# jacky121298/3DAL_PyTorch

Hardware: AMD Instinct MI355X
Metric: object-crops/sec through static+dynamic refinement heads (higher is better)
Workload: dtype f32; 1 GPU; StaticModelOneBoxEst forward+decode, 4096 crops x 1024 pts per GPU, fp32 (BASELINE.json configs[1]); items_per_gpu=4096, points_per_item=1024, sampler=device, parallelism=single GPU

## Files before the change

### 3dal_pytorch_amd/_hip.py

```python
import ctypes as C
import os

import numpy as np
import torch

_HERE = os.path.dirname(os.path.abspath(__file__))
LIB_PATH = os.path.join(_HERE, "lib3dal_hip.so")

OK, EINVAL, EWORKSPACE, EHIP = 0, -1, -2, -3
F32, BF16, F16, F16X3 = 0, 1, 2, 3
DTYPES = {"fp32": F32, "bf16": BF16, "fp16": F16, "f16x3": F16X3}
HEAD_INS_SEG, HEAD_STATIC_BOX_EST, HEAD_POINT_EMB, HEAD_BOX_EMB, HEAD_DYNAMIC_BOX_EST = range(5)
SAMPLER_DEVICE, SAMPLER_CHOICE = 0, 1
PHASE_SEG, PHASE_BOX, PHASE_ALL = 1, 2, 3

vp = C.c_void_p


class Layer(C.Structure):
    _fields_ = [("weight", vp), ("bias", vp), ("bn_weight", vp), ("bn_bias", vp), ("bn_mean", vp),
                ("bn_var", vp), ("c_in", C.c_int32), ("c_out", C.c_int32)]


class PackItem(C.Structure):
# ... 200 lines not shown
                ("out_indices", vp), ("out_key", vp), ("n_out", vp), ("status", vp), ("max_workgroups", C.c_int64),
                ("workspace", vp), ("workspace_bytes", C.c_size_t)]


class SpTableArgs(C.Structure):
    _fields_ = [("B", C.c_int64), ("in_shape", _i3), ("out_shape", _i3), ("kernel", _i3), ("stride", _i3), ("padding", _i3),
                ("reserved", C.c_int32), ("out_capacity", C.c_int64), ("n_out", vp), ("out_indices", vp), ("in_capacity", C.c_int64),
                ("n_in", vp), ("in_key", vp), ("in_pos", vp), ("table", vp), ("max_workgroups", C.c_int64)]


class SpConvArgs(C.Structure):
    _fields_ = [("taps", C.c_int32), ("c_in", C.c_int32), ("c_out", C.c_int32), ("relu", C.c_int32), ("center_tap", C.c_int32),
                ("reserved", C.c_int32), ("in_capacity", C.c_int64), ("x", vp), ("out_capacity", C.c_int64), ("n_out", vp),
                ("table", vp), ("packed", vp), ("residual", vp), ("y", vp), ("canvas", vp), ("out_indices", vp),
                ("canvas_B", C.c_int64), ("canvas_shape", _i3), ("reserved2", C.c_int32), ("status", vp),
                ("max_workgroups", C.c_int64)]


SP_WGRAD_SLICE = 1024


class SpTableTransposedArgs(C.Structure):
    _fields_ = [("B", C.c_int64), ("in_shape", _i3), ("out_shape", _i3), ("kernel", _i3), ("stride", _i3), ("padding", _i3),
                ("reserved", C.c_int32), ("in_capacity", C.c_int64), ("n_in", vp), ("in_indices", vp), ("out_capacity", C.c_int64),
                ("n_out", vp), ("out_key", vp), ("table", vp), ("max_workgroups", C.c_int64)]


class SpWgradArgs(C.Structure):
    _fields_ = [("taps", C.c_int32), ("c_in", C.c_int32), ("c_out", C.c_int32), ("reserved", C.c_int32), ("in_capacity", C.c_int64),
                ("x", vp), ("out_capacity", C.c_int64), ("n_out", vp), ("table", vp), ("dy", vp), ("dw", vp), ("db", vp),
                ("max_workgroups", C.c_int64), ("workspace", vp), ("workspace_bytes", C.c_size_t)]


ROI_OVERFLOW = 4096
ROI_MAX_TASKS, ROI_MAX_WIDTH = 16, 256
_f2 = C.c_float * 2


class BevGatherArgs(C.Structure):
    _fields_ = [("B", C.c_int64), ("H", C.c_int64), ("W", C.c_int64), ("C", C.c_int32), ("sample_index", C.c_int32), ("map", Map),
                ("n", C.c_int64), ("xy", vp), ("xy_stride", C.c_int64), ("sample", vp), ("pc_start", _f2), ("voxel_size", _f2),
                ("out_stride", C.c_float), ("points_per_row", C.c_int32), ("out", vp), ("out_row_stride", C.c_int64),
                ("out_col_offset", C.c_int64)]


class RoiShape(C.Structure):
    _fields_ = [("c_in", C.c_int32), ("n_shared", C.c_int32), ("n_cls", C.c_int32), ("n_reg", C.c_int32), ("shared", _i3),
                ("cls", _i3), ("reg", _i3), ("num_class", C.c_int32), ("code_size", C.c_int32)]


class RoiHeadArgs(C.Structure):
    _fields_ = [("shape", RoiShape), ("packed", vp), ("B", C.c_int64), ("M", C.c_int64), ("num_point", C.c_int32), ("C", C.c_int32),
                ("T", C.c_int32), ("box_cols", C.c_int32), ("K", C.c_int64), ("keep_stride", C.c_int64), ("boxes", vp), ("scores", vp),
                ("labels", vp), ("keep", vp), ("keep_count", vp), ("seg_offsets", vp), ("label_base", C.c_int32 * ROI_MAX_TASKS),
                ("bev", Map), ("H", C.c_int64), ("W", C.c_int64), ("pc_start", _f2), ("voxel_size", _f2), ("out_stride", C.c_float),
                ("rois", vp), ("roi_scores", vp), ("roi_features", vp), ("out_boxes", vp), ("out_scores", vp), ("out_labels", vp),
                ("out_counts", vp), ("out_features", vp), ("box_preds", vp), ("cls_preds", vp), ("status", vp), ("workspace", vp),
                ("workspace_bytes", C.c_size_t)]


ROI_NO_SAMPLE = 8192
ROI_CLS_SCORE = {"roi_iou": 0, "cls": 1}
ROI_TRAIN_MAX_M, ROI_TRAIN_MAX_R, ROI_TRAIN_MAX_G = 512, 512, 1024


class RoiTargetsArgs(C.Structure):
    _fields_ = [("B", C.c_int64), ("M", C.c_int64), ("R", C.c_int64), ("G", C.c_int64), ("code_size", C.c_int32),
                ("reserved0", C.c_int32), ("T", C.c_int32), ("reserved", C.c_int32), ("K", C.c_int64), ("keep_stride", C.c_int64),
                ("boxes", vp), ("scores", vp), ("labels", vp), ("keep", vp), ("keep_count", vp), ("seg_offsets", vp),
                ("label_base", C.c_int32 * ROI_MAX_TASKS), ("rois", vp), ("roi_scores", vp), ("roi_labels", vp), ("gt", vp),
                ("draws", vp), ("fg_per_image", C.c_int32), ("cls_score_type", C.c_int32), ("reg_fg_thresh", C.c_float),
                ("cls_fg_thresh", C.c_float), ("cls_bg_thresh", C.c_float), ("cls_bg_thresh_lo", C.c_float),
                ("cls_thresh_span", C.c_float), ("reserved2", C.c_float), ("hard_bg_ratio", C.c_double), ("slot", vp), ("sample", vp),
                ("out_rois", vp), ("out_labels", vp), ("out_scores", vp), ("gt_iou", vp), ("gt_src", vp), ("reg_valid", vp),
                ("cls_labels", vp), ("gt_of_rois", vp), ("out_boxes", vp), ("status", vp)]


CENTER_OVERFLOW = 16384
CENTER_MAX_OBJS, CENTER_MAX_CLASSES, CENTER_MAX_COLS = 1024, 64, 10
_pT = vp * ROI_MAX_TASKS


class CenterTargetsArgs(C.Structure):
    _fields_ = [("B", C.c_int64), ("G", C.c_int64), ("H", C.c_int64), ("W", C.c_int64), ("T", C.c_int32), ("max_objs", C.c_int32),
                ("num_class", C.c_int32 * ROI_MAX_TASKS), ("gt", vp), ("pc_start", _f2), ("voxel_size", _f2),
                ("out_size_factor", C.c_float), ("min_radius", C.c_int32), ("gaussian_overlap", C.c_double), ("hm", _pT),
                ("anno_box", _pT), ("ind", _pT), ("mask", _pT), ("cat", _pT), ("status", vp)]


class CenterLossArgs(C.Structure):
    _fields_ = [("B", C.c_int64), ("H", C.c_int64), ("W", C.c_int64), ("C", C.c_int32), ("n_cols", C.c_int32), ("max_objs", C.c_int32),
                ("reserved", C.c_int32), ("hm", Map), ("reg", Map), ("height", Map), ("dim", Map), ("rot", Map), ("vel", Map),
                ("target_hm", vp), ("anno_box", vp), ("ind", vp), ("mask", vp), ("cat", vp),
                ("code_weights", C.c_float * CENTER_MAX_COLS), ("weight", C.c_float), ("reserved2", C.c_float), ("out", vp),
                ("grad", vp), ("workspace", vp), ("workspace_bytes", C.c_size_t)]


AUG_TOO_MANY, AUG_OVERFLOW, AUG_BAD_ROW = 32768, 65536, 131072
AUG_MAX_BOXES, AUG_MAX_CAND = 1024, 64


class GtPasteArgs(C.Structure):
    _fields_ = [("B", C.c_int64), ("max_gt", C.c_int32), ("max_cand", C.c_int32), ("gt_boxes", vp), ("gt_classes", vp),
                ("gt_counts", vp), ("cand_boxes", vp), ("cand_group", vp), ("cand_counts", vp), ("accept", vp), ("coll", vp),
                ("status", vp)]


class AugmentPointsArgs(C.Structure):
    _fields_ = [("B", C.c_int64), ("n", C.c_int64), ("n_scene", C.c_int64), ("db_rows", C.c_int64), ("F", C.c_int32),
                ("transform", C.c_int32), ("max_cand", C.c_int64), ("scene", vp), ("scene_offsets", vp), ("db_points", vp),
                ("out_offsets", vp), ("cand_counts", vp), ("cand_seg_start", vp), ("cand_rows", vp), ("cand_db_row", vp),
                ("cand_boxes", vp), ("accept", vp), ("keys", vp), ("xform", vp), ("out", vp), ("status", vp),
                ("max_workgroups", C.c_int64), ("workspace", vp), ("workspace_bytes", C.c_size_t)]


class AugmentBoxesArgs(C.Structure):
    _fields_ = [("B", C.c_int64), ("max_gt", C.c_int32), ("max_cand", C.c_int32), ("max_objs", C.c_int32), ("n_classes", C.c_int32),
                ("transform", C.c_int32), ("reserved", C.c_int32), ("gt_boxes", vp), ("gt_classes", vp), ("gt_counts", vp),
                ("cand_boxes", vp), ("cand_classes", vp), ("cand_counts", vp), ("accept", vp), ("xform", vp),
                ("range", C.c_float * 4), ("out", vp), ("out_count", vp), ("status", vp)]


OPTIM_CHUNK, OPTIM_NORM_SPAN = 4096, 16384
OPTIM_TRUE_WD, OPTIM_CLIP, OPTIM_FUSED_ZERO = 1, 2, 4
(OPTIM_STEP, OPTIM_LR, OPTIM_BETA1, OPTIM_BETA2, OPTIM_EPS, OPTIM_WD, OPTIM_MAX_NORM, OPTIM_FLAGS, OPTIM_TOTAL_STEP,
 OPTIM_TABLE, OPTIM_SLOTS) = range(11)


class OptimChunk(C.Structure):
    _fields_ = [("param", vp), ("offset", C.c_int64), ("count", C.c_int32), ("decay", C.c_int32)]


_i, _i64, _u64, _sz = C.c_int, C.c_int64, C.c_uint64, C.c_size_t
SIGNATURES = {
    "dal3_version": (_i, []),
    "dal3_last_error": (C.c_char_p, []),
    "dal3_mean_size": (C.POINTER(C.c_float), []),
    "dal3_pack_weights": (_i, [_i, C.POINTER(Layer), _i, _i, vp, C.POINTER(_sz), vp]),
    "dal3_ins_seg_workspace_bytes": (_sz, [_i]),
    "dal3_ins_seg_plan_layout": (_i, [_i, C.POINTER(_sz), C.POINTER(_i)]),
    "dal3_ins_seg_encoder_route": (_i, [_i, _i, _i]),
    "dal3_ins_seg_forward": (_i, [vp, _i, _i, BCN, _i, _i, vp, vp, vp, vp, _sz, vp]),
    "dal3_ins_seg_encode": (_i, [vp, _i, _i, BCN, _i, _i, vp, vp]),
    "dal3_ins_seg_global_bias": (_i, [vp, _i, vp, _i, vp, vp]),
    "dal3_ins_seg_decode": (_i, [vp, _i, _i, BCN, _i, _i, vp, vp, vp, vp]),
    "dal3_gather_workspace_bytes": (_sz, [_i, _i]),
    "dal3_segment_counts": (_i, [vp, _i, _i, vp, vp]),
    "dal3_mask_compact_sample": (_i, [vp, BCN, _i, _i, _i, _i, _i, vp, _u64, _i64, vp, vp, vp, vp, _sz, vp]),
    "dal3_mask_compact_sample_step": (_i, [vp, BCN, _i, _i, _i, _i, _u64, vp, _i64, vp, vp, vp, vp, _sz, vp]),
    "dal3_point_head_workspace_bytes": (_sz, [_i]),
    "dal3_point_head_forward": (_i, [_i, vp, _i, BCN, _i, _i, vp, _i64, vp, _sz, vp]),
    "dal3_point_head_pool_workspace_bytes": (_sz, [_i, _i]),
    "dal3_point_head_screen_min_tiles": (_i, []),
    "dal3_point_head_screen_stride": (_i, []),
    "dal3_point_head_pool": (_i, [_i, vp, _i, BCN, _i, _i, vp, vp, vp, _sz, vp]),
    "dal3_dynamic_box_est_forward": (_i, [vp, vp, _i, vp, vp, _sz, vp]),
    "dal3_decode_boxes": (_i, [vp, _i, vp, _i64, _i, vp, _i64, vp, _i64, vp, vp, vp, vp, vp]),
    "dal3_recenter_rotz": (_i, [vp, _i, _i, vp, vp, vp, vp, vp, vp, vp]),
    "dal3_static_crop_prep": (_i, [vp, vp, vp, vp, vp, _i, _i, _u64, _i64, vp, vp, vp]),
    "dal3_dynamic_item_prep": (_i, [vp, vp, vp, vp, vp, vp, vp, vp, _i, _i, _i, _i, _u64, _i64, vp, vp, vp, vp]),
    "dal3_writeback_boxes": (_i, [vp, vp, vp, vp, vp, vp, vp, vp, vp, _i, _i64, vp, vp, vp]),
    "dal3_static_crop_labels": (_i, [vp, vp, vp, vp, _i, _i, _u64, _i64, vp, vp, vp]),
    "dal3_dynamic_item_labels": (_i, [vp, vp, vp, vp, vp, vp, vp, _i, _i, _i, _u64, _i64, vp, vp, vp, vp, vp]),
    "dal3_points_in_boxes": (_i, [vp, _i, _i64, _i64, vp, _i, _i, vp, vp]),
    "dal3_box_iou_pairwise": (_i, [vp, _i64, vp, _i64, _i, vp, vp, vp]),
    "dal3_box_iou_paired": (_i, [vp, vp, _i64, _i, vp, vp, vp]),
    "dal3_box_estimation_metrics": (_i, [C.POINTER(BoxMetricArgs), vp]),
    "dal3_track_workspace_bytes": (_sz, [_i64, _i64, _i64]),
    "dal3_track": (_i, [C.POINTER(TrackArgs), vp]),
    "dal3_track_match_workspace_bytes": (_sz, [_i64]),
    "dal3_track_match": (_i, [C.POINTER(TrackMatchArgs), vp]),
    "dal3_group_workspace_bytes": (_sz, [_i64, _i64]),
    "dal3_group_by_key": (_i, [C.POINTER(GroupArgs), vp]),
    "dal3_track_features": (_i, [C.POINTER(TrackFeatureArgs), vp]),
    "dal3_gt_table": (_i, [C.POINTER(GtTableArgs), vp]),
    "dal3_motion_classify_workspace_bytes": (_sz, [_i64]),
    "dal3_motion_classify": (_i, [C.POINTER(MotionClassifyArgs), vp]),
    "dal3_score_workspace_bytes": (_sz, [_i64]),
    "dal3_score_tracks": (_i, [C.POINTER(ScoreArgs), vp]),
    "dal3_best_gt_iou": (_i, [C.POINTER(BestGtArgs), vp]),
    "dal3_nms_workspace_bytes": (_sz, [_i64, _i]),
    "dal3_nms": (_i, [C.POINTER(NmsArgs), vp]),
    "dal3_center_decode_workspace_bytes": (_sz, [_i64, _i64, _i64]),
    "dal3_center_decode": (_i, [C.POINTER(CenterDecodeArgs), vp]),
    "dal3_center_decode_flip4_workspace_bytes": (_sz, [_i64, _i64, _i64]),
    "dal3_center_decode_flip4": (_i, [C.POINTER(CenterDecodeFlip4Args), vp]),
    "dal3_flip4_points": (_i, [vp, _i64, C.c_int32, vp, _i64, vp, vp, _i64, vp]),
    "dal3_voxelize_workspace_bytes": (_sz, [_i64, _i64]),
    "dal3_voxelize": (_i, [C.POINTER(VoxelizeArgs), vp]),
    "dal3_pillar_pack": (_i, [C.POINTER(Layer), _i, _i, C.c_double, vp, vp]),
    "dal3_pillar_features": (_i, [C.POINTER(PillarFeatureArgs), vp]),
    "dal3_pillar_scatter": (_i, [vp, vp, _i64, vp, _i, vp, _i64, _i64, _i64, vp]),
    "dal3_voxel_mean": (_i, [vp, vp, _i64, vp, _i, _i, vp, vp]),
    "dal3_conv2d_pack_floats": (_sz, [_i, _i, _i]),
    "dal3_conv2d_pack": (_i, [C.POINTER(Layer), _i, C.c_double, vp, vp]),
    "dal3_conv2d": (_i, [C.POINTER(Conv2dArgs), vp]),
    "dal3_sp_sort_workspace_bytes": (_sz, [_i64]),
    "dal3_sp_sort": (_i, [C.POINTER(SpSortArgs), vp]),
    "dal3_sp_downsample_workspace_bytes": (_sz, [_i64, _i]),
    "dal3_sp_downsample": (_i, [C.POINTER(SpDownsampleArgs), vp]),
    "dal3_sp_table": (_i, [C.POINTER(SpTableArgs), vp]),
    "dal3_sp_conv_pack_floats": (_sz, [_i, _i, _i]),
    "dal3_sp_conv_pack": (_i, [C.POINTER(Layer), _i, C.c_double, vp, vp, vp]),
    "dal3_sp_conv": (_i, [C.POINTER(SpConvArgs), vp]),
    "dal3_sp_table_transposed": (_i, [C.POINTER(SpTableTransposedArgs), vp]),
    "dal3_sp_wgrad_workspace_bytes": (_sz, [_i, _i, _i, _i64]),
    "dal3_sp_wgrad": (_i, [C.POINTER(SpWgradArgs), vp]),
    "dal3_bev_gather": (_i, [C.POINTER(BevGatherArgs), vp]),
    "dal3_box_points": (_i, [vp, _i64, _i, _i, vp, vp]),
    "dal3_roi_pack_floats": (_sz, [C.POINTER(RoiShape)]),
    "dal3_roi_pack": (_i, [C.POINTER(RoiShape), C.POINTER(Layer), _i, C.POINTER(C.c_double), vp, vp]),
    "dal3_roi_head_workspace_bytes": (_sz, [_i64, _i64, _i, _i, _i]),
    "dal3_roi_head": (_i, [C.POINTER(RoiHeadArgs), vp]),
    "dal3_roi_post": (_i, [vp, vp, vp, _i64, _i, vp, vp, vp]),
    "dal3_roi_targets": (_i, [C.POINTER(RoiTargetsArgs), vp]),
    "dal3_roi_loss": (_i, [vp, vp, _i64, _i, vp, vp, vp, C.POINTER(C.c_float), C.c_float, C.c_float, vp, vp, vp, vp]),
    "dal3_center_targets": (_i, [C.POINTER(CenterTargetsArgs), vp]),
    "dal3_center_loss_workspace_bytes": (_sz, [_i64, _i64, _i64, _i64]),
    "dal3_center_loss": (_i, [C.POINTER(CenterLossArgs), vp]),
    "dal3_gt_paste_select": (_i, [C.POINTER(GtPasteArgs), vp]),
    "dal3_augment_points_workspace_bytes": (_sz, [_i64, _i64]),
    "dal3_augment_points": (_i, [C.POINTER(AugmentPointsArgs), vp]),
    "dal3_augment_boxes": (_i, [C.POINTER(AugmentBoxesArgs), vp]),
    "dal3_optim_partials": (_i64, [_i64]),
    "dal3_optim_grad_norm": (_i, [vp, _i64, vp, vp, vp]),
    "dal3_optim_step": (_i, [vp, _i64, vp, vp, vp, _i64, vp, vp, vp]),
    "dal3_optim_total_norm": (_i, [vp, _i64, vp, vp]),
    "dal3_crop_workspace_bytes": (_sz, [_i64, _i64]),
    "dal3_crop_count": (_i, [vp, vp, vp, vp, vp, _i, _i64, _i64, vp, vp, _sz, vp]),
    "dal3_crop_fill": (_i, [vp, vp, vp, vp, vp, _i, _i64, _i64, vp, vp, vp, vp, vp, _i64, vp, _sz, vp]),
    "dal3_crop_starts": (_i, [vp, vp, _i64, vp, vp, vp]),
    "dal3_crop_starts_capped": (_i, [vp, vp, _i64, vp, vp, _i64, vp]),
    "dal3_tr_linear": (_i, [vp, _i64, _i, _i64, vp, vp, _i, vp, _i64, _i, vp, _i64, _i, vp, _i64, _i, vp, _sz, vp]),
    "dal3_tr_linear_workspace_bytes": (_sz, [_i, _i]),
    "dal3_tr_linear_pack_layout": (_i, [_i64, _i, _i64, _i, _i, _i]),
    "dal3_tr_pack_many": (_i, [vp, _i, vp]),
    "dal3_tr_linear_prepacked": (_i, [vp, _i64, _i, _i64, vp, vp, _i, vp, _i64, _i, vp, _i64, _i, vp, _i64, _i, vp, vp]),
    "dal3_tr_linear_x3_layout": (_i, [_i64, _i, _i64, _i, _i, _i]),
    "dal3_tr_linear_x3": (_i, [vp, _i64, _i, _i64, vp, vp, _i, vp, _i64, _i, vp, _i64, vp, vp, vp]),
    "dal3_tr_bnbwd_apply_amax": (_i, [vp, _i64, _i, _i64, vp, _i64, vp, vp, _i64, vp, vp, vp, vp, vp, vp, vp, vp, _i64, vp, vp]),
    "dal3_tr_colred_workspace_bytes": (_sz, [_i64, _i]),
    "dal3_tr_act_colsum": (_i, [vp, _i64, _i, _i64, vp, vp, _i, vp, _i64, vp, _sz, vp, vp]),
    "dal3_tr_colred": (_i, [vp, _i64, _i, _i64, _i, vp, _i64, vp, vp, _i64, vp, vp, vp, vp, vp, _sz, vp, vp]),
    "dal3_tr_pool_coef": (_i, [vp, vp, vp, vp, vp, vp, _i, _i, _i64, vp, vp, vp]),
    "dal3_tr_head2_forward": (_i, [vp, _i64, _i, _i64, vp, vp, _i, vp, _i64, _u64, vp, C.c_float, vp, _i64, vp, vp, vp]),
    "dal3_tr_head2_dgrad": (_i, [vp, _i64, _i, vp, _i64, _u64, vp, C.c_float, vp, _i64, vp, _i64, vp]),
    "dal3_tr_head2_dgrad_bnbwd": (_i, [vp, _i64, _i, vp, _i64, _u64, vp, C.c_float, vp, _i64, vp, _i64, vp, _i64, vp, vp, vp, vp, vp,
                                       vp, vp, vp, vp, vp, vp, _sz, vp]),
    "dal3_tr_head2_wgrad_workspace_bytes": (_sz, [_i64]),
    "dal3_tr_head2_wgrad": (_i, [vp, vp, _i64, _i, _i64, vp, vp, _i, vp, _i64, _u64, vp, C.c_float, vp, _sz, vp, vp]),
    "dal3_tr_conv1_workspace_bytes": (_sz, [_i64, _i]),
    "dal3_tr_conv1_bn_stats": (_i, [vp, _i64, _i64, _i, _i64, vp, _i64, vp, _i, vp, _i64, vp, vp, vp, vp, C.c_float, C.c_float, vp, vp,
                                    vp, vp, vp, _sz, vp]),
    "dal3_tr_conv1_wgrad": (_i, [vp, _i64, vp, _i64, _i, _i64, _i, vp, _sz, vp, vp]),
    "dal3_tr_gather_at": (_i, [vp, _i64, vp, _i64, _i, _i, vp, vp]),
    "dal3_tr_pool_zarg": (_i, [vp, vp, _i64, vp, _i64, vp, _i, _i, _i, _i, vp, vp]),
    "dal3_tr_pool_moments": (_i, [vp, _i64, vp, vp, vp, _i64, _i, _i, vp, vp]),
    "dal3_tr_pool_gv_workspace_bytes": (_sz, [_i]),
    "dal3_tr_pool_gv": (_i, [vp, vp, _i64, vp, _i, _i, vp, vp, vp, _sz, vp]),
    "dal3_tr_pool_dw": (_i, [vp, vp, _i64, vp, vp, vp, _i64, _i, vp, _i, _i, vp, vp]),
    "dal3_tr_pool_sparse": (_i, [vp, vp, vp, _i64, vp, _i64, _i, _i, _i, _i, vp, _i64, vp, vp]),
    "dal3_tr_box_loss": (_i, [vp] * 10 + [_i] + [vp] * 7),
    "dal3_tr_seg_ce_workspace_bytes": (_sz, [_i64]),
    "dal3_tr_seg_ce": (_i, [vp, vp, _i, _i64, vp, vp, vp, _sz, vp]),
    "dal3_tr_linear_red_workspace_bytes": (_sz, [_i64, _i]),
    "dal3_tr_linear_bn_stats": (_i, [vp, _i64, _i, _i64, vp, vp, _i, vp, _i64, vp, _i64, _i, vp, _i64, vp, _i64, vp, vp, vp, vp,
                                     C.c_float, C.c_float, vp, vp, vp, vp, vp, _sz, vp]),
    "dal3_tr_linear_bnbwd_sums": (_i, [vp, _i64, _i, _i64, vp, _i64, _i, vp, _i64, vp, _i64, vp, _i64, vp, vp, vp, vp, vp,
                                       vp, vp, vp, vp, vp, vp, _sz, vp]),
    "dal3_tr_bn_stats": (_i, [vp, _i64, _i, _i64, vp, vp, vp, vp, C.c_float, C.c_float, vp, vp, vp, vp, vp, _sz, vp]),
    "dal3_tr_bnbwd_sums": (_i, [vp, _i64, _i, _i64, vp, _i64, vp, vp, _i64, vp, vp, vp, vp, vp, vp, vp, vp, vp, vp, vp, _sz,
                                vp]),
    "dal3_tr_bn_finalize": (_i, [vp, _i, _i64, vp, vp, vp, vp, C.c_float, C.c_float, vp, vp, vp, vp, vp]),
    "dal3_tr_bnbwd_coef": (_i, [vp, _i, _i64, vp, vp, vp, vp, vp, vp, vp, vp]),
    "dal3_parse_box_pred": (_i, [vp, _i64, _i64, vp, vp, vp, vp, vp, vp, vp, vp]),
    "dal3_parse_box_pred_backward": (_i, [vp, vp, vp, vp, vp, vp, vp, _i64, vp, vp]),
    "dal3_tr_fc_max_rows": (_i, []),
    "dal3_tr_fc_max_act_cin": (_i, []),
    "dal3_tr_fc_forward": (_i, [vp, _i64, _i, _i64, vp, vp, _i, vp, _i64, _i, vp, _i, vp, _i64, vp, vp, vp, vp, C.c_float, C.c_float, vp, vp, vp, vp, vp]),
    "dal3_tr_fc_backward_w": (_i, [vp, _i64, _i64, _i, vp, _i64, vp, vp, vp, vp, vp, vp, vp, vp, _i, _i64, vp, vp, _i, vp, _i64, vp, _i64,
                                   vp, vp]),
    "dal3_tr_bnbwd_apply": (_i, [vp, _i64, _i, _i64, vp, _i64, vp, vp, _i64, vp, vp, vp, vp, vp, vp, vp, vp, _i64, vp]),
    "dal3_tr_bnbwd_apply_segsum_workspace_bytes": (_sz, [_i64, _i]),
    "dal3_tr_bnbwd_apply_segsum": (_i, [vp, _i64, _i, _i64, vp, _i64, vp, vp, vp, vp, vp, vp, vp, vp, _i64, _i64, vp, vp, _sz, vp]),
    "dal3_tr_wgrad_workspace_bytes": (_sz, [_i64, _i, _i]),
    "dal3_tr_wgrad": (_i, [vp, _i64, vp, _i64, vp, vp, _i, _i64, _i, _i, vp, _sz, vp, vp]),
    "dal3_tr_wgrad_final_many": (_i, [C.POINTER(WgradPart), _i, vp]),
    "dal3_tr_wgrad_x3_workspace_bytes": (_sz, [_i64, _i, _i]),
    "dal3_tr_wgrad_x3": (_i, [vp, _i64, vp, _i64, vp, vp, _i, vp, _i64, _i, _i, vp, _sz, vp, vp]),
    "dal3_tr_segmax": (_i, [vp, _i64, _i64, _i, vp, vp, vp, vp, _i64, vp, _sz, vp]),
    "dal3_tr_act_dropout": (_i, [vp, _i64, _i, _i64, vp, vp, _i, vp, _i64, _u64, vp, C.c_float, vp, _i64, vp]),
    "dal3_tr_linear_pool_workspace_bytes": (_sz, [_i, _i, _i64]),
    "dal3_tr_linear_pool": (_i, [vp, _i64, _i, _i64, vp, vp, _i, vp, _i64, vp, vp, vp, _i64, _i, vp, vp, vp, _sz, vp]),
    "dal3_tr_linear_pool_x3": (_i, [vp, _i64, _i, _i64, vp, vp, _i, vp, _i64, vp, vp, vp, _i64, _i, vp, vp, vp, _sz, vp]),
    "dal3_tr_linear_pool_x3_ok": (_i, [_i64, _i, _i64, _i]),
    "dal3_tr_segsum": (_i, [vp, _i64, _i64, _i, vp, _i64, vp]),
    "dal3_maxpool_n": (_i, [vp, _i64, _i64, vp, vp]),
    "dal3_maxpool_n_dtype": (_i, [vp, _i, _i64, _i64, vp, vp]),
    "dal3_shared_mlp_layer": (_i, [C.POINTER(Layer), _i, BCN, _i, _i, vp, vp, _sz, vp]),
    "dal3_shared_mlp_layer_workspace_bytes": (_sz, [_i, _i]),
    "dal3_static_workspace_bytes": (_sz, [_i, _i, _i]),
    "dal3_static_forward": (_i, [C.POINTER(StaticArgs), _i, vp]),
    "dal3_dynamic_workspace_bytes": (_sz, [_i, _i, _i]),
    "dal3_dynamic_forward": (_i, [C.POINTER(DynamicArgs), _i, vp]),
}

_lib = None


def lib():
    global _lib
    if _lib is None:
        if not os.path.exists(LIB_PATH):
            raise RuntimeError(
                f"{LIB_PATH} is missing: build the HIP library first "
                "(`make -C 3dal_pytorch_amd/csrc` or __graft_entry__.build()). "
                "There is no CPU/eager fallback for the eval-mode forward.")
        handle = C.CDLL(LIB_PATH)
        for name, (res, args) in SIGNATURES.items():
            fn = getattr(handle, name)
            fn.restype = res
            fn.argtypes = args
        from . import arch
        lib_mean = [handle.dal3_mean_size()[i] for i in range(9)]
        want = [C.c_float(v).value for row in arch.MEAN_SIZE for v in row]
        if lib_mean != want:
            raise RuntimeError(f"lib3dal_hip.so was built with MEAN_SIZE {lib_mean}, arch.MEAN_SIZE is {want}: rebuild the library")
        _lib = handle
    return _lib


def check(rc):
    if rc != OK:
        raise RuntimeError(f"lib3dal_hip error {rc}: {lib().dal3_last_error().decode()}")


def stream():
    return vp(torch.cuda.current_stream().cuda_stream)


def ptr(t):
    return vp(t.data_ptr()) if t is not None else vp(None)


def require_gpu(t, what):
    if not t.is_cuda:
        raise RuntimeError(
            f"{what} lives on {t.device}: the eval-mode forward runs only on an MI355X through "
            "lib3dal_hip.so (no CPU fallback). Move the model and its inputs to the GPU.")


def workspace(nbytes, device):
    return torch.empty(max(int(nbytes), 8), dtype=torch.uint8, device=device)


def host_offsets(offsets, n, name, sized_by, count):
    if torch.is_tensor(offsets):
        if offsets.is_cuda:
            raise TypeError(f"{name} must be on the host (a list, an array or a CPU tensor): {sized_by} from it, and "
                            "reading a device tensor back would be the synchronisation this call avoids")
        offsets = offsets.numpy()
    off = np.ascontiguousarray(np.asarray(offsets, dtype=np.int64).reshape(-1))
    if off.size < 1:
        raise ValueError(f"{name} needs {count} + 1 entries")
    if off[0] < 0 or off[-1] > n or np.any(np.diff(off) < 0):
        raise ValueError(f"{name} must be non-decreasing within [0, {n}]")
    return off


STORAGE = {torch.float32: F32, torch.bfloat16: BF16, torch.float16: F16}
BCN_NO_SMALL_JOB_KERNELS, BCN_NO_WORKLIST, BCN_NO_LDS_SAMPLER = 1, 2, 4
BCN_NO_DEC_PLAN = 16
BCN_NO_ENC_RESIDENT = 32
ENC_ROUTE_LATENCY, ENC_ROUTE_DENSE, ENC_ROUTE_TWO_LAUNCH, ENC_ROUTE_RESIDENT = 0, 1, 2, 3
DISPATCH_FLAGS = 0


def bcn(t):
    assert t.dim() == 3 and t.dtype in STORAGE
    sb, sc, sn = t.stride()
    return BCN(ptr(t), sb, sc, sn, STORAGE[t.dtype], DISPATCH_FLAGS)


def layer_struct(conv, bn):
    w = conv.weight
    c_in, c_out = getattr(conv, "in_channels", w.shape[1]), getattr(conv, "out_channels", w.shape[0])
    if not w.is_contiguous() or w.dtype != torch.float32:
        raise RuntimeError("weights must be contiguous fp32")
    L = Layer(ptr(w), ptr(conv.bias), None, None, None, None, c_in, c_out)
    if bn is not None:
        L.bn_weight, L.bn_bias = ptr(bn.weight), ptr(bn.bias)
        L.bn_mean, L.bn_var = ptr(bn.running_mean), ptr(bn.running_var)
    return L


def fold_layer_struct(conv, bn, what="the layer's parameters"):
    ts = [conv.weight] + ([conv.bias] if conv.bias is not None else [])
    if bn is not None:
        ts += [bn.weight, bn.bias, bn.running_mean, bn.running_var]
    for t in ts:
        require_gpu(t, what)
        if t.dtype != torch.float32 or not t.is_contiguous():
            raise RuntimeError("weights must be contiguous fp32")
    return layer_struct(conv, bn)


F16_MAX = 65504.0


def check_f16x3_range(pairs):
    with torch.no_grad():
        worst = None
        for conv, bn in pairs:
            w = conv.weight.detach().reshape(conv.weight.shape[0], -1).abs().amax(1)
            if bn is not None:
                w = w * (bn.weight.detach() / torch.sqrt(bn.running_var.detach() + 1e-5)).abs()
            m = w.max()
            worst = m if worst is None else torch.maximum(worst, m)
        if worst is not None and not float(worst) < F16_MAX:
            raise ValueError(f"precision 'f16x3': a folded weight of magnitude {float(worst):.3g} is beyond fp16's range "
                             f"({F16_MAX:g}); this head cannot run on the f16x3 kernels (use precision 'fp32')")


def pack(head_kind, pairs, device, dtype=F32):
    if dtype == F16X3:
        check_f16x3_range(pairs)
    arr = (Layer * len(pairs))(*[layer_struct(c, b) for c, b in pairs])
    need = _sz(0)
    check(lib().dal3_pack_weights(head_kind, arr, len(pairs), dtype, None, C.byref(need), None))
    buf = torch.empty(need.value, dtype=torch.uint8, device=device)
    assert buf.data_ptr() % 256 == 0
    check(lib().dal3_pack_weights(head_kind, arr, len(pairs), dtype, ptr(buf), C.byref(need), stream()))
    return buf
```

### 3dal_pytorch_amd/csrc/dal3_api.hip

```cpp
#include <stdarg.h>
#include <stdio.h>
#include <string.h>

#include <type_traits>

#include "dal3_block.h"
#include "dal3_kernels.h"
#include "dal3_lp.h"

static thread_local char g_err[512] = "";

static int fail(int code, const char* fmt, ...) {
    va_list ap;
    va_start(ap, fmt);
    vsnprintf(g_err, sizeof(g_err), fmt, ap);
    va_end(ap);
    return code;
}

#define HIP_TRY(expr)                                                                           \
    do {                                                                                        \
        hipError_t e_ = (expr);                                                                 \
        if (e_ != hipSuccess) return fail(DAL3_EHIP, "%s: %s", #expr, hipGetErrorString(e_)); \
    } while (0)
// ... 215 lines not shown
    const bool lp = dtype != DAL3_F32 && !x3;
    size_t floats;
    switch (head_kind) {
        case DAL3_HEAD_INS_SEG:
            floats = x3 ? measure(ins_seg_16_walk<InsSegX3W>) + DAL3_BLOB_TAIL_FLOATS
                        : lp ? measure(ins_seg_16_walk<InsSegLpW>) : measure(ins_seg_walk) + DAL3_BLOB_TAIL_FLOATS;
            break;
        case DAL3_HEAD_STATIC_BOX_EST:
        case DAL3_HEAD_POINT_EMB:
        case DAL3_HEAD_BOX_EMB:
            floats = x3 ? measure(point_head_16_walk, head_kind, true) + DAL3_BLOB_TAIL_FLOATS
                        : lp ? measure(point_head_16_walk, head_kind, false)
                             : measure(point_head_walk, head_kind) + DAL3_BLOB_TAIL_FLOATS;
            break;
        case DAL3_HEAD_DYNAMIC_BOX_EST: floats = measure(fc_head_walk); break;
        default: return fail(DAL3_EINVAL, "dal3_pack_weights: unknown head_kind %d", head_kind);
    }
    const size_t need = floats * sizeof(float);
    if (!packed_dev) {
        *bytes_inout = need;
        return 0;
    }
    if (*bytes_inout < need) return fail(DAL3_EWORKSPACE, "dal3_pack_weights: need %zu bytes, got %zu", need, *bytes_inout);
    if (!L) return fail(DAL3_EINVAL, "dal3_pack_weights: layers is NULL");
    if (reinterpret_cast<uintptr_t>(packed_dev) & 255) return fail(DAL3_EINVAL, "packed_dev must be 256-byte aligned");
    hipStream_t s = static_cast<hipStream_t>(stream);
    HIP_TRY(hipMemsetAsync(packed_dev, 0, need, s));

    if (head_kind == DAL3_HEAD_INS_SEG) {
        if (n_layers != 10) return fail(DAL3_EINVAL, "ins_seg expects 10 layers, got %d", n_layers);
        const int c_in = L[0].c_in;
        if (c_in != 3 && c_in != 4) return fail(DAL3_EINVAL, "ins_seg c_in must be 3 or 4, got %d", c_in);
        static const int co[10] = {64, 64, 64, 128, 1024, 512, 256, 128, 128, 2};
        static const int ci[10] = {0, 64, 64, 64, 128, 1088, 512, 256, 128, 128};
        for (int i = 0; i < 10; ++i) TRY(check_layer(L[i], i == 0 ? c_in : ci[i], co[i], "ins_seg layer"));
        const int64_t F = 512;
        if (x3) {
            const InsSegX3W w = view(packed_dev, ins_seg_16_walk<InsSegX3W>);
            uint16_t* enc = const_cast<uint16_t*>(w.enc_stream);
            uint16_t* dec = const_cast<uint16_t*>(w.dec_stream);
            TRY(pack_ins_seg_16_open(L, c_in, w, true, s));
            HIP_TRY(launch_pack_weight_x3(L[1], 0, 0, 64, 2, 2, enc, s));
            HIP_TRY(launch_pack_weight_x3(L[2], 0, 0, 64, 2, 2, enc + 16 * F, s));
            HIP_TRY(launch_pack_weight_x3(L[3], 0, 0, 64, 4, 2, enc + 32 * F, s));
            HIP_TRY(launch_pack_weight_x3(L[4], 0, 0, 128, 32, 4, enc + 64 * F, s));
            HIP_TRY(launch_pack_weight_x3(L[1], 0, 0, 64, 2, 2, dec, s));
            HIP_TRY(launch_pack_weight_x3(L[5], 0, 0, 64, 16, 2, dec, s, PackGroups{2, 16 * F, 24 * F, 40 * F}));
            HIP_TRY(launch_pack_weight_x3(L[6], 1, 0, 512, 8, 16, dec, s, PackGroups{8, 32 * F, 72 * F, 40 * F, 624 * F}));
            HIP_TRY(launch_pack_weight_x3(L[7], 0, 0, 256, 4, 8, dec + 656 * F, s));
            HIP_TRY(launch_pack_weight_x3(L[8], 0, 0, 128, 4, 4, dec + 784 * F, s));
            HIP_TRY(launch_pack_weight_x3(L[9], 0, 0, 128, 1, 4, dec + 848 * F, s));
            return 0;
        }
        if (lp) {
            const InsSegLpW w = view(packed_dev, ins_seg_16_walk<InsSegLpW>);
            uint16_t* enc = const_cast<uint16_t*>(w.enc_stream);
            uint16_t* dec = const_cast<uint16_t*>(w.dec_stream);
            TRY(pack_ins_seg_16_open(L, c_in, w, false, s));
            HIP_TRY(launch_pack_weight_lp(L[1], dtype, 0, 0, 64, 2, 2, enc, s));
            HIP_TRY(launch_pack_weight_lp(L[2], dtype, 0, 0, 64, 2, 2, enc + 8 * F, s));
            HIP_TRY(launch_pack_weight_lp(L[3], dtype, 0, 0, 64, 4, 2, enc + 16 * F, s));
            HIP_TRY(launch_pack_weight_lp(L[4], dtype, 0, 0, 128, 32, 4, enc + 32 * F, s));
            HIP_TRY(launch_pack_weight_lp(L[1], dtype, 0, 0, 64, 2, 2, dec, s));
            HIP_TRY(launch_pack_weight_lp(L[5], dtype, 0, 0, 64, 16, 2, dec, s, PackGroups{2, 8 * F, 40 * F, 20 * F}));
            HIP_TRY(launch_pack_weight_lp(L[6], dtype, 1, 0, 512, 8, 16, dec, s, PackGroups{8, 44 * F, 64 * F, 20 * F}));
            HIP_TRY(launch_pack_weight_lp(L[7], dtype, 0, 0, 256, 4, 8, dec, s, PackGroups{16, 360 * F, 400 * F, 40 * F}));
            HIP_TRY(launch_pack_weight_lp(L[8], dtype, 0, 0, 128, 4, 4, dec + 440 * F, s));
            HIP_TRY(launch_pack_weight_lp(L[9], dtype, 0, 0, 128, 1, 4, dec + 472 * F, s));
            return 0;
        }
        const InsSegW w = view(packed_dev, ins_seg_walk);
        HIP_TRY(launch_pack_weight(L[0], PACK_FIRST, 0, c_in, 2, 2, mut(w.w1), s));
        HIP_TRY(launch_pack_bias(L[0], mut(w.b1), s));
        TRY(pack_frag(L[1], PACK_FRAG_MT_MAJOR, 0, 64, w.enc_stream, ENC_W2, w.b2, s));
        TRY(pack_frag(L[2], PACK_FRAG_MT_MAJOR, 0, 64, w.enc_stream, ENC_W3, w.b3, s));
        TRY(pack_frag(L[3], PACK_FRAG_MT_MAJOR, 0, 64, w.enc_stream, ENC_W4, w.b4, s));
        TRY(pack_frag(L[4], PACK_FRAG_MT_MAJOR, 0, 128, w.enc_stream, ENC_W5, w.b5, s));
        TRY(pack_frag(L[1], PACK_FRAG_MT_MAJOR, 0, 64, w.dec_stream, DEC_W2, nullptr, s));
        TRY(pack_frag(L[5], PACK_FRAG_MT_MAJOR, 0, 64, w.dec_stream, DEC_MIX, w.db1, s,
                      PackGroups{ 2, 0, 8 * 256, 40 * 256}));
        HIP_TRY(launch_pack_weight(L[5], PACK_ROWMAJOR, 64, 1024, 0, 0, mut(w.dw1g), s));
        TRY(pack_frag(L[6], PACK_FRAG_KT_MAJOR, 0, 512, w.dec_stream, DEC_MIX, w.db2, s,
                      PackGroups{ 8, 16 * 256, 56 * 256, 40 * 256}));
        TRY(pack_frag(L[7], PACK_FRAG_MT_MAJOR, 0, 256, w.dec_stream, DEC_W3, w.db3, s));
        TRY(pack_frag(L[8], PACK_FRAG_MT_MAJOR, 0, 128, w.dec_stream, DEC_W4, w.db4, s));
        TRY(pack_frag(L[5], PACK_FRAG_MT_MAJOR, 0, 64, w.lat_stream, LAT_W1A, nullptr, s));
        TRY(pack_frag(L[6], PACK_FRAG_MT_MAJOR, 0, 512, w.lat_stream, LAT_W2, nullptr, s));
        HIP_TRY(launch_pack_weight(L[9], PACK_ROWMAJOR, 0, 128, 0, 0, mut(w.dw5), s));
        HIP_TRY(launch_pack_bias(L[9], mut(w.db5), s));
        HIP_TRY(launch_pack_weight(L[4], PACK_ROWMAJOR, 0, 128, 0, 0, mut(w.w5row), s));
        HIP_TRY(launch_pack_weight_lp(L[4], DAL3_F16, 0, 0, 128, 32, 4, reinterpret_cast<uint16_t*>(mut(w.w5h)), s));
        HIP_TRY(launch_pack_screen_bound(L[4], mut(w.scr_pq), const_cast<int32_t*>(w.scr_flag), s));
        int32_t* dec_flag = const_cast<int32_t*>(w.dec_flag);
        HIP_TRY(launch_pack_dec_chain(L[6], w.db2, mut(w.dw2c), dec_flag, s));
        HIP_TRY(launch_pack_dec_chain(L[7], w.db3, mut(w.dw3c), dec_flag, s));
        HIP_TRY(launch_pack_dec_chain(L[8], w.db4, mut(w.dw4c), dec_flag, s));
        HIP_TRY(launch_pack_weight_lp(L[5], DAL3_F16, 0, 0, 64, 16, 2, reinterpret_cast<uint16_t*>(mut(w.w1h)), s));
        HIP_TRY(launch_pack_dec_prune(L[5], mut(w.dw1c), mut(w.prn_pq), const_cast<uint32_t*>(w.dec_ident),
                                      const_cast<int32_t*>(w.prn_flag), s));
        return 0;
    }
    if (head_kind == DAL3_HEAD_DYNAMIC_BOX_EST) {
        if (n_layers != 3) return fail(DAL3_EINVAL, "dynamic box_est expects 3 layers, got %d", n_layers);
        return pack_fc(L, view(packed_dev, fc_head_walk), s);
    }
    int c_in, ks, c[4], n_fc, fi[3], fo[3];
    point_head_dims(head_kind, &c_in, &ks, c, &n_fc, fi, fo);
    if (n_layers != 4 + n_fc) return fail(DAL3_EINVAL, "head %d expects %d layers, got %d", head_kind, 4 + n_fc, n_layers);
    TRY(check_layer(L[0], c_in, c[0], "conv1"));
    for (int i = 1; i < 4; ++i) TRY(check_layer(L[i], c[i - 1], c[i], "conv"));
    if (x3 || lp) {
        const PointHeadLpW w = view(packed_dev, point_head_16_walk, head_kind, x3);
        TRY(pack_head_open(L, c_in, ks, c[0], w.w1, w.b1, w.bias, w.bias + c[1], w.bias + c[1] + c[2], s));
        uint16_t* st = const_cast<uint16_t*>(w.stream);
        const int64_t SEGE = (int64_t)LP_HEAD_SEG * 512;
        int64_t off = 0;
        int seg = 0;
        for (int l = 1; l < 4; ++l) {
            const int kt = c[l - 1] / 32, mt = c[l] / 32;
            if (x3) {
                HIP_TRY(launch_pack_weight_x3(L[l], 0, 0, c[l - 1], mt, kt, st + off, s));
                off += (int64_t)mt * kt * 2048;
            } else {
                const int tps = lp_tps(kt, mt);
                HIP_TRY(launch_pack_weight_lp(L[l], dtype, 0, 0, c[l - 1], mt, kt, st, s,
                                              PackGroups{tps * kt, seg * SEGE, (seg + 1) * SEGE, SEGE}));
                seg += mt / tps;
            }
        }
        return pack_fc(L + 4, w.fc, s);
    }
    const PointHeadW w = view(packed_dev, point_head_walk, head_kind);
    TRY(pack_head_open(L, c_in, ks, c[0], w.w1, w.b1, w.b2, w.b3, w.b4, s));
    const int f3 = (c[1] / 32) * (c[0] / 32) * 4, f4 = f3 + (c[2] / 32) * (c[1] / 32) * 4;
    TRY(pack_frag(L[1], PACK_FRAG_MT_MAJOR, 0, c[0], w.stream, 0, nullptr, s));
    TRY(pack_frag(L[2], PACK_FRAG_MT_MAJOR, 0, c[1], w.stream, f3, nullptr, s));
    TRY(pack_frag(L[3], PACK_FRAG_MT_MAJOR, 0, c[2], w.stream, f4, nullptr, s));
    if (w.w4row) {
        HIP_TRY(launch_pack_weight(L[3], PACK_ROWMAJOR, 0, 256, 0, 0, mut(w.w4row), s));
        HIP_TRY(launch_pack_weight_lp(L[3], DAL3_F16, 0, 0, 256, 16, 8, reinterpret_cast<uint16_t*>(mut(w.w4h)), s));
        HIP_TRY(launch_pack_screen_bound(L[3], mut(w.scr_pq), const_cast<int32_t*>(w.scr_flag), s));
    }
    return pack_fc(L + 4, w.fc, s);
}

static BCN to_bcn(const dal3_bcn& t) { return BCN{t.data, t.stride_b, t.stride_c, t.stride_n, t.dtype, t.flags}; }

static int check_bcn(const dal3_bcn& t, const char* what) {
    if (!t.data) return fail(DAL3_EINVAL, "%s: null data pointer", what);
    if (t.stride_n <= 0 || t.stride_c <= 0) return fail(DAL3_EINVAL, "%s: strides must be positive", what);
    if (t.dtype != DAL3_F32 && t.dtype != DAL3_BF16 && t.dtype != DAL3_F16)
        return fail(DAL3_EINVAL, "%s: storage dtype %d is none of DAL3_F32 / DAL3_BF16 / DAL3_F16", what, t.dtype);
    if (t.dtype != DAL3_F32 && (reinterpret_cast<uintptr_t>(t.data) & 1)) return fail(DAL3_EINVAL, "%s: 16-bit data must be 2-byte aligned", what);
    if (t.flags & ~(DAL3_BCN_NO_SMALL_JOB_KERNELS | DAL3_BCN_NO_WORKLIST | DAL3_BCN_NO_LDS_SAMPLER | DAL3_BCN_NO_DEC_PLAN | DAL3_BCN_NO_ENC_RESIDENT)) return fail(DAL3_EINVAL, "%s: unknown bits in flags (%d)", what, t.flags);
    return 0;
}

static int check_extent(int64_t B, int64_t N, const char* what) {
    if (B <= 0 || N <= 0) return fail(DAL3_EINVAL, "%s: B and N must be positive (B=%lld N=%lld)", what, (long long)B, (long long)N);
    if (B > DAL3_MAX_ITEMS) return fail(DAL3_EINVAL, "%s: B=%lld items exceed DAL3_MAX_ITEMS (%d)", what, (long long)B, DAL3_MAX_ITEMS);
    if (N > DAL3_MAX_POINTS_PER_ITEM)
        return fail(DAL3_EINVAL, "%s: N=%lld points per item exceed DAL3_MAX_POINTS_PER_ITEM (%d)", what, (long long)N, DAL3_MAX_POINTS_PER_ITEM);
    if (B * ((N + 31) / 32) > (int64_t)DAL3_MAX_TILES)
        return fail(DAL3_EINVAL, "%s: B=%lld x N=%lld is %lld 32-point tiles, more than DAL3_MAX_TILES (%d): split the batch", what,
                    (long long)B, (long long)N, (long long)(B * ((N + 31) / 32)), DAL3_MAX_TILES);
    return 0;
}

struct InsSegWs { float* g; float* gb; uint32_t* prune; uint32_t* plan_k; float* plan_gbc; int32_t* plan_nch; };
static InsSegWs carve_ins_seg(Carver& c, int B) {
    InsSegWs w;
    w.g = c.take<float>((size_t)B * 1024);
    w.gb = c.take<float>((size_t)B * 512);
    w.prune = c.take<uint32_t>((size_t)B * 513);
    w.plan_k = c.take<uint32_t>((size_t)B * DEC_PLAN_LD);
    w.plan_gbc = c.take<float>((size_t)B * 512);
    w.plan_nch = c.take<int32_t>((size_t)B);
    return w;
}
extern "C" size_t dal3_ins_seg_workspace_bytes(int B) {
    Carver c(nullptr, 0);
    carve_ins_seg(c, B);
    return c.off;
}

extern "C" int dal3_ins_seg_plan_layout(int B, size_t off[4], int* min_dead) {
    if (B <= 0 || !off) return fail(DAL3_EINVAL, "ins_seg_plan_layout: bad argument");
    char* const origin = reinterpret_cast<char*>(uintptr_t(4096));
    Carver c(origin, ~size_t(0));
    const InsSegWs w = carve_ins_seg(c, B);
    off[0] = reinterpret_cast<char*>(w.prune) - origin, off[1] = reinterpret_cast<char*>(w.plan_k) - origin;
    off[2] = reinterpret_cast<char*>(w.plan_gbc) - origin, off[3] = reinterpret_cast<char*>(w.plan_nch) - origin;
    if (min_dead) *min_dead = DAL3_DEC_MIN_DEAD;
    return 0;
}

extern "C" int dal3_ins_seg_encoder_route(int B, int N, int flags) {
    TRY(check_extent(B, N, "ins_seg_encoder_route"));
    if (flags & ~(DAL3_BCN_NO_SMALL_JOB_KERNELS | DAL3_BCN_NO_WORKLIST | DAL3_BCN_NO_LDS_SAMPLER | DAL3_BCN_NO_DEC_PLAN | DAL3_BCN_NO_ENC_RESIDENT))
        return fail(DAL3_EINVAL, "ins_seg_encoder_route: unknown bits in flags (%d)", flags);
    return enc_route(flags, B, N);
}

static int check_dtype(int dtype) {
    if (dtype != DAL3_F32 && dtype != DAL3_BF16 && dtype != DAL3_F16 && dtype != DAL3_F16X3)
        return fail(DAL3_EINVAL, "unknown dtype %d", dtype);
    return 0;
}

static int ins_seg_run(const void* packed, int dtype, int c_in, const dal3_bcn& pts, int B, int N, float* logits,
                       uint8_t* mask, float* global_feat_out, const InsSegWs& ws, hipStream_t s) {
    TRY(check_dtype(dtype));
    if (!packed || !logits || !mask) return fail(DAL3_EINVAL, "ins_seg: null pointer");
    TRY(check_extent(B, N, "ins_seg"));
    if (c_in != 3 && c_in != 4) return fail(DAL3_EINVAL, "ins_seg: c_in must be 3 or 4");
    TRY(check_bcn(pts, "pts"));
    const BCN x = to_bcn(pts);
    HIP_TRY(launch_nonfinite_rows(x, B, N, c_in, ws.g, 1024, s));
    if (dtype == DAL3_F32) {
        const InsSegW w = view(packed, ins_seg_walk);
        const bool plan = dec_plan_route(x.flags, B, N);
        if (plan) HIP_TRY(hipMemsetAsync(ws.prune, 0, (size_t)B * 513 * sizeof(uint32_t), s));
        HIP_TRY(launch_ins_seg_encode(w, x, c_in, B, N, ws.g, s, plan ? ws.prune : nullptr));
        HIP_TRY(launch_fc(w.dw1g, w.db1, ws.g, 1024, ws.gb, 512, B, 1024, 512, 0, s));
        if (plan) HIP_TRY(launch_dec_plan(w, ws.gb, ws.prune, B, ws.plan_k, ws.plan_gbc, ws.plan_nch, s));
        HIP_TRY(launch_ins_seg_decode(w, x, c_in, B, N, ws.gb, logits, mask, s,
                                      plan ? DecPlan{ws.plan_k, ws.plan_gbc, ws.plan_nch} : DecPlan{nullptr, nullptr, nullptr}));
    } else if (dtype == DAL3_F16X3) {
        const InsSegX3W w = view(packed, ins_seg_16_walk<InsSegX3W>);
        HIP_TRY(launch_ins_seg_encode_x3(w, x, c_in, B, N, ws.g, s));
        HIP_TRY(launch_fc(w.dw1g, w.db1, ws.g, 1024, ws.gb, 512, B, 1024, 512, 0, s));
        HIP_TRY(launch_ins_seg_decode_x3(w, x, c_in, B, N, ws.gb, logits, mask, s));
    } else {
        const InsSegLpW w = view(packed, ins_seg_16_walk<InsSegLpW>);
        HIP_TRY(launch_ins_seg_encode_lp(dtype, w, x, c_in, B, N, ws.g, s));
        HIP_TRY(launch_fc(w.dw1g, w.db1, ws.g, 1024, ws.gb, 512, B, 1024, 512, 0, s));
        HIP_TRY(launch_ins_seg_decode_lp(dtype, w, x, c_in, B, N, ws.gb, logits, mask, s));
    }
    if (global_feat_out)
        HIP_TRY(hipMemcpyAsync(global_feat_out, ws.g, (size_t)B * 1024 * sizeof(float), hipMemcpyDeviceToDevice, s));
    return 0;
}

extern "C" int dal3_ins_seg_forward(const void* packed, int dtype, int c_in, dal3_bcn pts, int B, int N, float* logits,
                                    uint8_t* mask, float* global_feat_out, void* workspace, size_t workspace_bytes,
                                    dal3_stream stream) {
    if (!workspace) return fail(DAL3_EINVAL, "ins_seg: workspace is NULL");
    TRY(check_extent(B, N, "ins_seg"));
    Carver c(workspace, workspace_bytes);
    const InsSegWs ws = carve_ins_seg(c, B);
    if (!c.ok) return fail(DAL3_EWORKSPACE, "ins_seg: workspace needs %zu bytes, got %zu", c.off, workspace_bytes);
    return ins_seg_run(packed, dtype, c_in, pts, B, N, logits, mask, global_feat_out, ws, static_cast<hipStream_t>(stream));
}

extern "C" int dal3_ins_seg_encode(const void* packed, int dtype, int c_in, dal3_bcn pts, int B, int N,
                                   float* global_feat, dal3_stream stream) {
    TRY(check_dtype(dtype));
    if (!packed || !global_feat || (c_in != 3 && c_in != 4)) return fail(DAL3_EINVAL, "ins_seg_encode: bad argument");
    TRY(check_extent(B, N, "ins_seg_encode"));
    TRY(check_bcn(pts, "pts"));
    hipStream_t s = static_cast<hipStream_t>(stream);
    if (dtype == DAL3_F32)
        HIP_TRY(launch_ins_seg_encode(view(packed, ins_seg_walk), to_bcn(pts), c_in, B, N,
                                      global_feat, s));
    else if (dtype == DAL3_F16X3)
        HIP_TRY(launch_ins_seg_encode_x3(view(packed, ins_seg_16_walk<InsSegX3W>), to_bcn(pts), c_in, B, N, global_feat, s));
    else
        HIP_TRY(launch_ins_seg_encode_lp(dtype, view(packed, ins_seg_16_walk<InsSegLpW>), to_bcn(pts), c_in, B, N, global_feat, s));
    return 0;
}

extern "C" int dal3_ins_seg_global_bias(const void* packed, int dtype, const float* global_feat, int B, float* gbias,
                                        dal3_stream stream) {
    TRY(check_dtype(dtype));
    if (!packed || !global_feat || !gbias) return fail(DAL3_EINVAL, "ins_seg_global_bias: bad argument");
    TRY(check_extent(B, 1, "ins_seg_global_bias"));
    const float *dw1g, *db1;
    auto sections = [&](const auto& w) { dw1g = w.dw1g, db1 = w.db1; };
    if (dtype == DAL3_F32) sections(view(packed, ins_seg_walk));
    else if (dtype == DAL3_F16X3) sections(view(packed, ins_seg_16_walk<InsSegX3W>));
    else sections(view(packed, ins_seg_16_walk<InsSegLpW>));
    HIP_TRY(launch_fc(dw1g, db1, global_feat, 1024, gbias, 512, B, 1024, 512, 0, static_cast<hipStream_t>(stream)));
    return 0;
}

extern "C" int dal3_ins_seg_decode(const void* packed, int dtype, int c_in, dal3_bcn pts, int B, int N,
                                   const float* gbias, float* logits, uint8_t* mask, dal3_stream stream) {
    TRY(check_dtype(dtype));
    if (!packed || !gbias || !logits || !mask || (c_in != 3 && c_in != 4)) return fail(DAL3_EINVAL, "ins_seg_decode: bad argument");
    TRY(check_extent(B, N, "ins_seg_decode"));
    TRY(check_bcn(pts, "pts"));
    hipStream_t s = static_cast<hipStream_t>(stream);
    if (dtype == DAL3_F32)
        HIP_TRY(launch_ins_seg_decode(view(packed, ins_seg_walk), to_bcn(pts), c_in, B, N,
                                      gbias, logits, mask, s));
    else if (dtype == DAL3_F16X3)
        HIP_TRY(launch_ins_seg_decode_x3(view(packed, ins_seg_16_walk<InsSegX3W>), to_bcn(pts), c_in, B, N, gbias, logits, mask, s));
    else
        HIP_TRY(launch_ins_seg_decode_lp(dtype, view(packed, ins_seg_16_walk<InsSegLpW>), to_bcn(pts), c_in, B, N, gbias, logits, mask, s));
    return 0;
}

extern "C" size_t dal3_gather_workspace_bytes(int B, int N) {
    Carver c(nullptr, 0);
    c.take<int32_t>((size_t)B * N);
    return c.off;
}

extern "C" int dal3_segment_counts(const uint8_t* mask, int B, int N, int32_t* counts, dal3_stream stream) {
    if (!mask || !counts) return fail(DAL3_EINVAL, "segment_counts: bad argument");
    TRY(check_extent(B, N, "segment_counts"));
    HIP_TRY(launch_segment_counts(mask, B, N, counts, static_cast<hipStream_t>(stream)));
    return 0;
}

static int gather_run(const uint8_t* mask, const dal3_bcn& pts, int B, int N, int C, int M, int sampler,
                      const int32_t* choice, uint64_t seed, int64_t item_offset, int32_t* counts, int32_t* obj_idx,
                      float* obj_pts, int32_t* pos, hipStream_t s, const int64_t* step = nullptr) {
    if (!mask || !counts || !obj_idx || !obj_pts) return fail(DAL3_EINVAL, "gather: null pointer");
    if (M <= 0 || C <= 0 || C > 8) return fail(DAL3_EINVAL, "gather: bad shape");
    TRY(check_extent(B, N, "gather"));
    TRY(check_extent(B, M, "gather (object points)"));
    if (sampler == DAL3_SAMPLER_CHOICE && !choice) return fail(DAL3_EINVAL, "gather: DAL3_SAMPLER_CHOICE needs choice");
    if (sampler != DAL3_SAMPLER_CHOICE && sampler != DAL3_SAMPLER_DEVICE) return fail(DAL3_EINVAL, "gather: bad sampler");
    TRY(check_bcn(pts, "pts"));
    HIP_TRY(launch_compact_sample(mask, to_bcn(pts), B, N, C, M, sampler, choice, seed, item_offset, counts, pos,
                                  obj_idx, obj_pts, s, step));
    return 0;
}

extern "C" int dal3_mask_compact_sample(const uint8_t* mask, dal3_bcn pts, int B, int N, int C, int M, int sampler,
                                        const int32_t* choice, uint64_t seed, int64_t item_offset, int32_t* counts,
                                        int32_t* obj_idx, float* obj_pts, void* workspace, size_t workspace_bytes,
                                        dal3_stream stream) {
    if (!workspace) return fail(DAL3_EINVAL, "gather: workspace is NULL");
    TRY(check_extent(B, N, "gather"));
    Carver c(workspace, workspace_bytes);
    int32_t* pos = c.take<int32_t>((size_t)B * N);
    if (!c.ok) return fail(DAL3_EWORKSPACE, "gather: workspace needs %zu bytes, got %zu", c.off, workspace_bytes);
    return gather_run(mask, pts, B, N, C, M, sampler, choice, seed, item_offset, counts, obj_idx, obj_pts, pos,
                      static_cast<hipStream_t>(stream));
}

extern "C" int dal3_mask_compact_sample_step(const uint8_t* mask, dal3_bcn pts, int B, int N, int C, int M, uint64_t seed,
                                             const int64_t* step, int64_t item_offset, int32_t* counts, int32_t* obj_idx,
                                             float* obj_pts, void* workspace, size_t workspace_bytes, dal3_stream stream) {
    if (!workspace) return fail(DAL3_EINVAL, "gather: workspace is NULL");
    TRY(check_extent(B, N, "gather"));
    Carver c(workspace, workspace_bytes);
    int32_t* pos = c.take<int32_t>((size_t)B * N);
    if (!c.ok) return fail(DAL3_EWORKSPACE, "gather: workspace needs %zu bytes, got %zu", c.off, workspace_bytes);
    return gather_run(mask, pts, B, N, C, M, DAL3_SAMPLER_DEVICE, nullptr, seed, item_offset, counts, obj_idx, obj_pts, pos,
                      static_cast<hipStream_t>(stream), step);
}

#define HEAD_WORK_MAX_POINTS 2560
struct HeadWs { float* feat; float* t1; float* t2; void* work; size_t work_bytes; };
static HeadWs carve_head(Carver& c, int B) {
    HeadWs w;
    w.feat = c.take<float>((size_t)B * 512);
    w.t1 = c.take<float>((size_t)B * 512);
    w.t2 = c.take<float>((size_t)B * 512);
    w.work_bytes = point_head_worklist_bytes(B, HEAD_WORK_MAX_POINTS);
    w.work = c.take<char>(w.work_bytes);
    return w;
}
extern "C" size_t dal3_point_head_workspace_bytes(int B) {
    Carver c(nullptr, 0);
    carve_head(c, B);
    return c.off;
}

static int fc_chain(const FcW& f, const float* x, int64_t xs, float* out, int64_t out_stride, int B, float* t1,
                    float* t2, hipStream_t s, const DecodeArgs* dec = nullptr) {
    const float* cur = x;
    int64_t cs = xs;
    for (int i = 0; i < f.n; ++i) {
        const bool last = i == f.n - 1;
        float* dst = last ? out : (i % 2 == 0 ? t1 : t2);
        const int64_t ds = last ? out_stride : f.c_out[i];
        if (last && dec) {
            if (f.c_out[i] != 39 || out_stride != 39 || dec->box_pred != out || f.relu[i])
                return fail(DAL3_EINVAL, "fc_chain: a fused decode needs the 39-wide box_pred layer last");
            HIP_TRY(launch_fc39_decode(f.w[i], f.b[i], cur, cs, B, f.c_in[i], *dec, s));
            return 0;
        }
        HIP_TRY(launch_fc(f.w[i], f.b[i], cur, cs, dst, ds, B, f.c_in[i], f.c_out[i], f.relu[i], s));
        cur = dst;
        cs = ds;
    }
    return 0;
}

static int point_head_run(int head_kind, const void* packed, int dtype, const dal3_bcn& x, int B, int M, float* out,
                          int64_t out_stride, const HeadWs& ws, hipStream_t s, const int32_t* distinct = nullptr,
                          const DecodeArgs* dec = nullptr) {
    TRY(check_dtype(dtype));
    if (head_kind != DAL3_HEAD_STATIC_BOX_EST && head_kind != DAL3_HEAD_POINT_EMB && head_kind != DAL3_HEAD_BOX_EMB)
        return fail(DAL3_EINVAL, "point_head: head_kind %d is not a point head", head_kind);
    if (!packed || !out) return fail(DAL3_EINVAL, "point_head: null pointer");
    TRY(check_extent(B, M, "point_head"));
    TRY(check_bcn(x, "x"));
    int c_in, ks, c[4], n_fc, fi[3], fo[3];
    point_head_dims(head_kind, &c_in, &ks, c, &n_fc, fi, fo);
    if (dtype == DAL3_F16X3) {
        const PointHeadX3W w = view(packed, point_head_16_walk, head_kind, true);
        HIP_TRY(launch_point_head_x3(head_kind, w, to_bcn(x), c_in, B, M, ws.feat, distinct, s));
        return fc_chain(w.fc, ws.feat, 512, out, out_stride, B, ws.t1, ws.t2, s, dec);
    }
    if (dtype != DAL3_F32) {
        const PointHeadLpW w = view(packed, point_head_16_walk, head_kind, false);
        HIP_TRY(launch_point_head_lp(dtype, head_kind, w, to_bcn(x), c_in, B, M, ws.feat, distinct, s));
        return fc_chain(w.fc, ws.feat, 512, out, out_stride, B, ws.t1, ws.t2, s, dec);
    }
    const PointHeadW w = view(packed, point_head_walk, head_kind);
    HIP_TRY(launch_point_head(head_kind, w, to_bcn(x), c_in, B, M, ws.feat, distinct, s, ws.work, ws.work_bytes));
    return fc_chain(w.fc, ws.feat, 512, out, out_stride, B, ws.t1, ws.t2, s, dec);
}

extern "C" int dal3_point_head_forward(int head_kind, const void* packed, int dtype, dal3_bcn x, int B, int M, float* out,
                                       int64_t out_stride, void* workspace, size_t workspace_bytes,
                                       dal3_stream stream) {
    if (!workspace) return fail(DAL3_EINVAL, "point_head: workspace is NULL");
    TRY(check_extent(B, M, "point_head"));
    Carver c(workspace, workspace_bytes);
    const HeadWs ws = carve_head(c, B);
    if (!c.ok) return fail(DAL3_EWORKSPACE, "point_head: workspace needs %zu bytes, got %zu", c.off, workspace_bytes);
    return point_head_run(head_kind, packed, dtype, x, B, M, out, out_stride, ws, static_cast<hipStream_t>(stream));
}

extern "C" size_t dal3_point_head_pool_workspace_bytes(int B, int M) {
    return B > 0 && M > 0 ? point_head_worklist_bytes(B, M) : 0;
}

extern "C" int dal3_point_head_pool(int head_kind, const void* packed, int dtype, dal3_bcn x, int B, int M,
                                    const int32_t* n_distinct, float* feat, void* workspace, size_t workspace_bytes,
                                    dal3_stream stream) {
    TRY(check_dtype(dtype));
    if (head_kind != DAL3_HEAD_STATIC_BOX_EST && head_kind != DAL3_HEAD_POINT_EMB && head_kind != DAL3_HEAD_BOX_EMB)
        return fail(DAL3_EINVAL, "point_head_pool: head_kind %d is not a point head", head_kind);
    if (!packed || !feat) return fail(DAL3_EINVAL, "point_head_pool: null pointer");
    if (workspace && (reinterpret_cast<uintptr_t>(workspace) & 15)) return fail(DAL3_EINVAL, "point_head_pool: workspace must be 16-byte aligned");
    TRY(check_extent(B, M, "point_head_pool"));
    TRY(check_bcn(x, "x"));
    hipStream_t s = static_cast<hipStream_t>(stream);
    int c_in, ks, c[4], n_fc, fi[3], fo[3];
    point_head_dims(head_kind, &c_in, &ks, c, &n_fc, fi, fo);
    if (dtype == DAL3_F16X3) {
        HIP_TRY(launch_point_head_x3(head_kind, view(packed, point_head_16_walk, head_kind, true), to_bcn(x), c_in, B, M, feat, n_distinct, s));
        return 0;
    }
    if (dtype != DAL3_F32) {
        const PointHeadLpW w = view(packed, point_head_16_walk, head_kind, false);
        HIP_TRY(launch_point_head_lp(dtype, head_kind, w, to_bcn(x), c_in, B, M, feat, n_distinct, s));
        return 0;
    }
    const PointHeadW w = view(packed, point_head_walk, head_kind);
    HIP_TRY(launch_point_head(head_kind, w, to_bcn(x), c_in, B, M, feat, n_distinct, s, workspace, workspace_bytes));
    return 0;
}

extern "C" int dal3_point_head_screen_min_tiles(void) { return DAL3_HEAD_SCREEN ? DAL3_HEAD_SCR_MIN_TILES : 0x7fffffff; }
extern "C" int dal3_point_head_screen_stride(void) { return DAL3_HEAD_SCR_STRIDE; }

extern "C" int dal3_dynamic_box_est_forward(const void* packed, const float* embedding, int B, float* box_pred,
                                            void* workspace, size_t workspace_bytes, dal3_stream stream) {
    if (!packed || !embedding || !box_pred || !workspace) return fail(DAL3_EINVAL, "dynamic_box_est: bad argument");
    TRY(check_extent(B, 1, "dynamic_box_est"));
    Carver c(workspace, workspace_bytes);
    const HeadWs ws = carve_head(c, B);
    if (!c.ok) return fail(DAL3_EWORKSPACE, "dynamic_box_est: workspace needs %zu bytes, got %zu", c.off, workspace_bytes);
    return fc_chain(view(packed, fc_head_walk), embedding, 384, box_pred, 39, B, ws.t1, ws.t2,
                    static_cast<hipStream_t>(stream));
}

extern "C" int dal3_decode_boxes(float* box_pred, int B, const float* center_add, int64_t center_add_stride,
                                 int center_inplace, const float* boxes_center_add, int64_t boxes_center_add_stride,
                                 const float* yaw_base, int64_t yaw_stride, float* heading_residuals,
                                 float* size_residuals, float* center, float* boxes7, dal3_stream stream) {
    if (!box_pred || B <= 0) return fail(DAL3_EINVAL, "decode_boxes: bad argument");
    HIP_TRY(launch_decode_boxes(box_pred, B, center_add, center_add_stride, center_inplace, boxes_center_add,
                                boxes_center_add_stride, yaw_base, yaw_stride, heading_residuals, size_residuals,
                                center, boxes7, static_cast<hipStream_t>(stream)));
    return 0;
}

extern "C" int dal3_recenter_rotz(const float* obj_pts, int B, int M, const float* init_box7, const float* box_one7,
                                  const float* bbox_gt7, float* obj_pts_two, int64_t* heading_class_label,
                                  float* heading_residual_label, dal3_stream stream) {
    if (!obj_pts || !init_box7 || !box_one7 || !obj_pts_two || B <= 0 || M <= 0)
        return fail(DAL3_EINVAL, "recenter_rotz: bad argument");
    if (bbox_gt7 && (!heading_class_label || !heading_residual_label))
        return fail(DAL3_EINVAL, "recenter_rotz: bbox_gt given without label outputs");
    HIP_TRY(launch_recenter(obj_pts, B, M, init_box7, box_one7, bbox_gt7, obj_pts_two, heading_class_label,
                            heading_residual_label, static_cast<hipStream_t>(stream)));
    return 0;
}

extern "C" int dal3_static_crop_prep(const double* points, const int64_t* offsets, const int32_t* choice,
                                     const double* pose, const double* box, int B, int N, uint64_t seed,
                                     int64_t item_offset, float* pts_out, float* init_box_out, dal3_stream stream) {
    if (!points || !offsets || !pose || !box || !pts_out || !init_box_out || B <= 0 || N < 7)
        return fail(DAL3_EINVAL, "static_crop_prep: bad argument (N must be >= 7)");
    HIP_TRY(launch_static_crop_prep(points, offsets, choice, pose, box, B, N, seed, item_offset, pts_out, init_box_out,
                                    static_cast<hipStream_t>(stream)));
    return 0;
}

extern "C" int dal3_dynamic_item_prep(const double* points, const int64_t* frame_offsets, const double* boxes,
                                      const int64_t* track_first, const int32_t* item_track, const int32_t* item_frame,
                                      const int32_t* choice, const double* pose, int B, int n_per, int r, int s,
                                      uint64_t seed, int64_t item_offset, float* pts_out, float* box_out,
                                      float* init_box_out, dal3_stream stream) {
    if (!points || !frame_offsets || !boxes || !track_first || !item_track || !item_frame || !pose || !pts_out ||
        !box_out || !init_box_out || B <= 0 || n_per <= 0 || r < 0 || s < 0)
        return fail(DAL3_EINVAL, "dynamic_item_prep: bad argument");
    HIP_TRY(launch_dynamic_item_prep(points, frame_offsets, boxes, track_first, item_track, item_frame, choice, pose, B,
                                     n_per, r, s, seed, item_offset, pts_out, box_out, init_box_out,
                                     static_cast<hipStream_t>(stream)));
    return 0;
}

extern "C" int dal3_static_crop_labels(const double* points, const int64_t* offsets, const int32_t* choice,
                                       const double* pose, int B, int N, uint64_t seed, int64_t item_offset,
                                       const double* gt_planes, uint8_t* mask_label, dal3_stream stream) {
    if (!points || !offsets || !pose || !gt_planes || !mask_label || B <= 0 || N <= 0)
        return fail(DAL3_EINVAL, "static_crop_labels: bad argument");
    HIP_TRY(launch_static_crop_labels(points, offsets, choice, pose, B, N, seed, item_offset, gt_planes, mask_label,
                                      static_cast<hipStream_t>(stream)));
    return 0;
}

extern "C" int dal3_dynamic_item_labels(const double* points, const int64_t* frame_offsets, const int64_t* track_first,
                                        const int32_t* item_track, const int32_t* item_frame, const int32_t* choice,
                                        const double* pose, int B, int n_per, int r, uint64_t seed, int64_t item_offset,
                                        const double* xform, const double* planes, const uint8_t* valid,
                                        uint8_t* mask_label, dal3_stream stream) {
    if (!points || !frame_offsets || !track_first || !item_track || !item_frame || !pose || !xform || !planes || !valid ||
        !mask_label || B <= 0 || n_per <= 0 || r < 0)
        return fail(DAL3_EINVAL, "dynamic_item_labels: bad argument");
    HIP_TRY(launch_dynamic_item_labels(points, frame_offsets, track_first, item_track, item_frame, choice, pose, B, n_per, r,
                                       seed, item_offset, xform, planes, valid, mask_label,
                                       static_cast<hipStream_t>(stream)));
    return 0;
}

extern "C" int dal3_points_in_boxes(const void* points, int points_f64, int64_t P, int64_t stride, const double* planes,
                                    int K, int f32_math, uint8_t* inside, dal3_stream stream) {
    if (P < 0 || K < 0 || stride < 3 || ((P > 0 && K > 0) && (!points || !planes || !inside)))
        return fail(DAL3_EINVAL, "points_in_boxes: bad argument (stride must be >= 3)");
    if (points_f64 && f32_math) return fail(DAL3_EINVAL, "points_in_boxes: float32 arithmetic needs float32 points");
    HIP_TRY(launch_points_in_boxes(points, points_f64, P, stride, planes, K, f32_math, inside,
                                   static_cast<hipStream_t>(stream)));
    return 0;
}

static int box_iou_args_ok(const char* what, const void* a, int64_t n, const void* b, int64_t m, int boxes_f64,
                           const float* iou_bev, const float* iou_3d, int64_t blocks) {
    if (n < 0 || m < 0 || (boxes_f64 != 0 && boxes_f64 != 1))
        return fail(DAL3_EINVAL, "%s: bad argument (n, m >= 0, boxes_f64 0 or 1)", what);
    if (n > DAL3_MAX_ITEMS || m > DAL3_MAX_ITEMS)
        return fail(DAL3_EINVAL, "%s: more than DAL3_MAX_ITEMS boxes on one side; split the call", what);
    if (blocks > DAL3_MAX_TILES) return fail(DAL3_EINVAL, "%s: launch grid beyond DAL3_MAX_TILES; split the call", what);
    if (!iou_bev && !iou_3d) return fail(DAL3_EINVAL, "%s: no output (iou_bev and iou_3d both NULL)", what);
    if (n > 0 && m > 0 && (!a || !b)) return fail(DAL3_EINVAL, "%s: null boxes", what);
    return 0;
}

extern "C" int dal3_box_iou_pairwise(const void* a, int64_t n, const void* b, int64_t m, int boxes_f64, float* iou_bev,
                                     float* iou_3d, dal3_stream stream) {
    const int64_t blocks = (n >= 0 && m >= 0 && n <= DAL3_MAX_ITEMS && m <= DAL3_MAX_ITEMS) ? box_iou_pairwise_blocks(n, m) : 0;
    TRY(box_iou_args_ok("box_iou_pairwise", a, n, b, m, boxes_f64, iou_bev, iou_3d, blocks));
    HIP_TRY(launch_box_iou_pairwise(a, n, b, m, boxes_f64, iou_bev, iou_3d, static_cast<hipStream_t>(stream)));
    return 0;
}

extern "C" int dal3_box_iou_paired(const void* a, const void* b, int64_t n, int boxes_f64, float* iou_bev, float* iou_3d,
                                   dal3_stream stream) {
    const int64_t blocks = (n >= 0 && n <= DAL3_MAX_ITEMS) ? box_iou_paired_blocks(n) : 0;
    TRY(box_iou_args_ok("box_iou_paired", a, n, b, n, boxes_f64, iou_bev, iou_3d, blocks));
    HIP_TRY(launch_box_iou_paired(a, b, n, boxes_f64, iou_bev, iou_3d, static_cast<hipStream_t>(stream)));
    return 0;
}

extern "C" int dal3_box_estimation_metrics(const dal3_box_metric_args* args, dal3_stream stream) {
    if (!args) return fail(DAL3_EINVAL, "box_estimation_metrics: null args");
    const dal3_box_metric_args& a = *args;
    if (a.B < 0 || a.N < 0 || a.B > DAL3_MAX_ITEMS || a.N > DAL3_MAX_POINTS_PER_ITEM)
        return fail(DAL3_EINVAL, "box_estimation_metrics: bad B / N (0 <= B <= DAL3_MAX_ITEMS, 0 <= N <= DAL3_MAX_POINTS_PER_ITEM)");
    if (!a.acc && !a.iou_bev && !a.iou_3d) return fail(DAL3_EINVAL, "box_estimation_metrics: no accumulator and no output");
    if ((a.f64_fields & ~255) || (a.i32_fields & ~3))
        return fail(DAL3_EINVAL, "box_estimation_metrics: unknown bits in f64_fields / i32_fields");
    if (a.B > 0) {
        const void* need[10] = {a.center, a.heading_scores, a.heading_residuals, a.size_scores, a.size_residuals,
                                a.center_label, a.heading_class_label, a.heading_residual_label, a.size_class_label,
                                a.size_residual_label};
        const int64_t ld[10] = {a.ld_center, a.ld_heading_scores, a.ld_heading_residuals, a.ld_size_scores,
                                a.ld_size_residuals, a.ld_center_label, a.ld_heading_class_label,
                                a.ld_heading_residual_label, a.ld_size_class_label, a.ld_size_residual_label};
        for (int k = 0; k < 10; ++k) {
            if (!need[k]) return fail(DAL3_EINVAL, "box_estimation_metrics: null field %d", k);
            if (ld[k] < 0) return fail(DAL3_EINVAL, "box_estimation_metrics: negative row stride of field %d", k);
        }
    }
    if (a.logits) {
        if (!a.acc) return fail(DAL3_EINVAL, "box_estimation_metrics: the segmentation term needs the accumulator");
        if (a.B > 0 && a.N > 0 && !a.mask_label) return fail(DAL3_EINVAL, "box_estimation_metrics: null mask_label");
        if (a.mask_dtype != DAL3_MASK_U8 && a.mask_dtype != DAL3_MASK_F32)
            return fail(DAL3_EINVAL, "box_estimation_metrics: mask_dtype must be DAL3_MASK_U8 or DAL3_MASK_F32");
        if (a.logits_stride_b < 0 || a.logits_stride_n < 0 || a.logits_stride_c < 0 || a.mask_stride_b < 0 ||
            a.mask_stride_n < 0)
            return fail(DAL3_EINVAL, "box_estimation_metrics: negative stride");
        if (1 + a.B * box_estimation_metrics_chunks(a.N) > DAL3_MAX_TILES)
            return fail(DAL3_EINVAL, "box_estimation_metrics: launch grid beyond DAL3_MAX_TILES; split the call");
    }
    HIP_TRY(launch_box_estimation_metrics(args, static_cast<hipStream_t>(stream)));
// ... 1709 lines not shown
```

### 3dal_pytorch_amd/csrc/dal3_head_screen.hip

```cpp
#include "dal3_device.h"
#include "dal3_kernels.h"
#include "dal3_lp.h"
#include "dal3_screen.h"

#ifndef HEAD_SCR_CAP
#define HEAD_SCR_CAP 1024
#endif
#define HEAD_SCR_XLD 132
#define HEAD_SCR_SW 16
#ifndef HEAD_SCR_DEPTH
#define HEAD_SCR_DEPTH 1
#endif
#define HEAD_SCR_XMAX_BITS 0x476A6000
#ifndef HEAD_RUN
#define HEAD_RUN 6
#endif

#ifdef DAL3_SCREEN_COUNT
__device__ unsigned long long g_head_scr_count[8];
extern "C" int dal3_debug_head_screen_counts(unsigned long long* out, int reset) {
    hipError_t e = hipMemcpyFromSymbol(out, HIP_SYMBOL(g_head_scr_count), sizeof(g_head_scr_count));
    if (e == hipSuccess && reset) {
        unsigned long long z[8] = {};
        e = hipMemcpyToSymbol(HIP_SYMBOL(g_head_scr_count), z, sizeof(z));
    }
    return (int)e;
}
#define HSCR_COUNT(k, v)                                                    \
    do {                                                                    \
        if (lane == 0) atomicAdd(&g_head_scr_count[k], (unsigned long long)(v)); \
    } while (0)
#else
#define HSCR_COUNT(k, v)
#endif

#ifdef DAL3_STAMP
__device__ unsigned long long* g_head_stamps = nullptr;
extern "C" int dal3_debug_set_head_stamps(void* p) {
    return (int)hipMemcpyToSymbol(HIP_SYMBOL(g_head_stamps), &p, sizeof(p));
}
#define HSTAMP_NOW(t)                                                               \
    do {                                                                            \
        __builtin_amdgcn_sched_barrier(0);                                          \
        asm volatile("s_memtime %0\n\ts_waitcnt lgkmcnt(0)" : "=s"(t)::"memory"); \
        __builtin_amdgcn_sched_barrier(0);                                          \
    } while (0)
#define HSTAMP(k)                                \
    do {                                         \
        unsigned long long t_;                   \
        HSTAMP_NOW(t_);                          \
        st_acc[k] += (uint32_t)(t_ - st_prev);   \
        st_prev = t_;                            \
    } while (0)
#define HSTAMP_ADD(k, v) st_acc[k] += (v)
#else
#define HSTAMP(k)
#define HSTAMP_ADD(k, v)
#endif

template <int KS, int C1, int C2, int C3>
__global__ __launch_bounds__(64) void point_head_screen_kernel(PointHeadW w, BCN x, int c_in, float* __restrict__ feat,
                                                               uint32_t* __restrict__ ctl, const u32x4* __restrict__ list) {
    constexpr int T = 1;
    constexpr int KT = C3 / 32;
    static_assert(C3 == 256, "the bound, the two halves of k and the fp16 fragments are laid out for conv4 256 -> 512");
    const int lane = threadIdx.x & 63;
    const int h = lane >> 5;
    __shared__ float s_b4[512];
    __shared__ int s_run[512];
    __shared__ int s_g[512];
    __shared__ f32x2 s_pq[512];
    __shared__ uint32_t s_list[HEAD_SCR_CAP];
    __shared__ float s_part[HEAD_SCR_CAP];
    __shared__ __attribute__((aligned(16))) float s_x[32 * HEAD_SCR_XLD];
    __shared__ __attribute__((aligned(16))) uint32_t s_stage[64 * (HEAD_SCR_SW + 4)];
    static_assert(4 * (3 * 512 * 4 + 512 * 8 + HEAD_SCR_CAP * 8 + 32 * HEAD_SCR_XLD * 4 + 64 * (HEAD_SCR_SW + 4) * 4) <= 160 * 1024,
                  "the screened head's LDS exceeds a quarter of a CU's 160 KiB: lower HEAD_SCR_CAP, HEAD_SCR_XLD or HEAD_SCR_SW");
    static_assert(16 * 64 <= 64 * (HEAD_SCR_SW + 4), "the stage holds the hit words of conv4's 16 blocks");
    for (int i = threadIdx.x; i < 512; i += 64) {
        s_b4[i] = w.b4[i];
        s_run[i] = 0;
        s_pq[i] = reinterpret_cast<const f32x2*>(w.scr_pq)[i];
    }
    __syncthreads();
    const uint32_t n_live = ctl[0];
    uint32_t run0 = n_live / (2u * gridDim.x);
    run0 = run0 < 1u ? 1u : (run0 > HEAD_RUN ? HEAD_RUN : run0);
    const uint32_t first_free = gridDim.x * run0;
    uint32_t cur = blockIdx.x * run0, run_end = cur + run0;
    if (cur >= n_live) return;
    const bool blob_dense = *w.scr_flag != 0;

    constexpr uint32_t FRAGS23 = ((C2 / 32) * (C1 / 32) + (C3 / 32) * (C2 / 32)) * 4u;
    WRing<DAL3_PF, true> ring;
    ring.init(w.stream, lane, FRAGS23 * 1024u);
    WRing<8> r16;
    r16.init(w.w4h, lane);
    f32x16 bias = tile_from_channels(w.b2, h);
    u32x4 e = list[cur];
    float in[T][KS];
    load_points<KS, T>(x, (int64_t)e[0], (int)e[1] * 32, (int)e[2], c_in, in, lane);
    auto enter = [&](int64_t b) {
        const int* gi = reinterpret_cast<const int*>(feat + b * 512);
#pragma unroll
        for (int c = lane; c < 512; c += 64) s_g[c] = __hip_atomic_load(gi + c, __ATOMIC_RELAXED, __HIP_MEMORY_SCOPE_AGENT);
    };
    auto flush = [&](int64_t b) {
        int* gi = reinterpret_cast<int*>(feat + b * 512);
#pragma unroll
        for (int c = lane; c < 512; c += 64) {
            const int v = s_run[c];
            if (v > 0) atomicMax(gi + c, v);
            s_run[c] = 0;
        }
    };
    auto dense_tile = [&](const f32x16 (&x3)[T][KT]) {
        WRing<DAL3_PF> r32;
        r32.init(w.stream + FRAGS23 * 64, lane);
        conv_max_layer<KT, T>(r32, s_b4, x3, reinterpret_cast<float*>(s_run), 16, lane);
    };
    enter((int64_t)e[0]);
#ifdef DAL3_STAMP
    uint32_t st_acc[10] = {};
    unsigned long long st_prev;
    HSTAMP_NOW(st_prev);
#endif
    for (;;) {
        const int64_t b = (int64_t)e[0];
        const int e_t = (int)e[1], e_n = (int)e[2];
        const bool last_of_run = cur + 1 >= run_end || cur + 1 >= n_live;
        uint32_t nxt = 0, take = 1;
        if (last_of_run) {
            const uint32_t left = n_live > run_end ? n_live - run_end : 0u;
            take = left / (2u * gridDim.x);
            take = take < 1u ? 1u : (take > HEAD_RUN ? HEAD_RUN : take);
            if (lane == 0) nxt = atomicAdd(&ctl[1], take);
        }
        f32x16 x3[T][KT];
        float in_n[T][KS];
        uint32_t ncur, nend;
        {
            f32x16 x1[T][C1 / 32], x2[T][C2 / 32];
            first_layer<KS, C1 / 32, T>(w.w1, w.b1, in, x1, lane);
            mlp_layer_ring<C1 / 32, C2 / 32, T>(ring, w.b2, w.b3, bias, x1, x2, lane);
            if (last_of_run) {
                ncur = (uint32_t)__builtin_amdgcn_readfirstlane((int)nxt) + first_free;
                nend = ncur + take;
            } else {
                ncur = cur + 1;
                nend = run_end;
            }
            const uint32_t nclamp = ncur < n_live ? ncur : cur;
            e = list[nclamp];
            mlp_layer_ring<C2 / 32, C3 / 32, T>(ring, w.b3, w.b2, bias, x2, x3, lane);
            load_points<KS, T>(x, (int64_t)e[0], (int)e[1] * 32, (int)e[2], c_in, in_n, lane);
        }
        HSCR_COUNT(0, 1);
        HSTAMP(0);
        HSTAMP_ADD(8, 1u);

        int xm = 0;
#pragma unroll
        for (int kt = 0; kt < KT; ++kt) {
#pragma unroll
            for (int r = 0; r < 16; ++r) {
                const int v = __float_as_int(x3[0][kt][r]);
                xm = v > xm ? v : xm;
            }
        }
        if (blob_dense || __builtin_amdgcn_ballot_w64(xm > HEAD_SCR_XMAX_BITS) != 0) {
            HSCR_COUNT(1, 1);
            dense_tile(x3);
            HSTAMP(7);
        } else {
            float ss = 0.0f;
#pragma unroll
            for (int kt = 0; kt < KT; ++kt) {
#pragma unroll
                for (int r = 0; r < 16; ++r) ss = fmaf(x3[0][kt][r], x3[0][kt][r], ss);
            }
            ss += __shfl_xor(ss, 32);
#pragma unroll
            for (int d = 16; d >= 1; d >>= 1) ss = __builtin_fmaxf(ss, __shfl_xor(ss, d));
            const float X = sqrtf(ss) * (1.0f + 0x1p-15f);

            ActTile<FP16> xh[KT];
#pragma unroll
            for (int kt = 0; kt < KT; ++kt) xh[kt] = pack_relu<FP16>(x3[0][kt]);

            ScreenHits<T> hits;
            hits.init();
            uint32_t vmask = 0;
            {
                const int left = e_n - e_t * 32;
#pragma unroll
                for (int r = 0; r < 16; ++r) vmask |= tile_chan(r, h) < left ? (1u << (15 - r)) : 0u;
            }
            HSTAMP(1);
            auto block_const = [&](int mt) -> float {
                const int c = 32 * mt + (lane & 31);
                const f32x2 pq = s_pq[c];
                float E = fmaf(X, pq[0], pq[1]);
                E = fmaf(E, 0x1p-20f, E);
                const int gs = s_g[c], gr = s_run[c];
                const float G = __int_as_float(gs > gr ? gs : gr), bb = s_b4[c];
                if (bits_nonfinite(G)) return 3.0e38f;
                return (G - bb) - fmaf(__builtin_fabsf(G) + __builtin_fabsf(bb), 0x1p-22f, E);
            };
            uint32_t hb = 0;
            auto ep_slice = [&](const f32x16& acc, int i, float k) {
                hb = scr_push_hit(hb, acc[2 * i], k);
                hb = scr_push_hit(hb, acc[2 * i + 1], k);
            };
            auto ep_finish = [&](int mt) {
                hits.park_block(s_stage, mt, hb & vmask, lane);
            };
            auto mm = [&](f32x16& acc, int mt, auto side) {
                acc = f32x16{};
#pragma unroll
                for (int i = 0; i < 2 * KT; ++i) {
                    const f16x8_t a = __builtin_bit_cast(f16x8_t, r16.slot[i & 7]);
                    r16.slot[i & 7] = r16.fetch_at(((16u * (uint32_t)mt + (uint32_t)i + 8u) & 255u) * 1024u);
                    acc = FP16::mfma(xh[i >> 1].k[i & 1], a, acc);
                    DAL3_SCHED_FENCE();
                    side(i);
                    DAL3_SCHED_FENCE();
                }
            };
            f32x16 accA, accB;
            float kA = block_const(0), kB;
            mm(accA, 0, NoSide());
            int mt = 1;
            for (; mt + 1 < 16; mt += 2) {
                kB = block_const(mt);
                mm(accB, mt, [&](int i) { if (i < 8) ep_slice(accA, i, kA); });
                ep_finish(mt - 1);
                kA = block_const(mt + 1);
                mm(accA, mt + 1, [&](int i) { if (i < 8) ep_slice(accB, i, kB); });
                ep_finish(mt);
            }
            kB = block_const(mt);
            mm(accB, mt, [&](int i) { if (i < 8) ep_slice(accA, i, kA); });
            ep_finish(mt - 1);
#pragma unroll
            for (int i = 0; i < 8; ++i) ep_slice(accB, i, kB);
            ep_finish(mt);
            HSTAMP(2);
            uint32_t cnt1[T];
            const bool overflow = scr_build_lists<T, 16, HEAD_SCR_CAP>(s_stage, s_list, hits, cnt1, lane);
            const uint32_t cnt = cnt1[0];
            HSCR_COUNT(3, cnt);
            HSTAMP(3);

            if (overflow) {
                HSCR_COUNT(2, 1);
                dense_tile(x3);
                HSTAMP(7);
            } else {
#pragma unroll
                for (int half = 0; half < 2; ++half) {
                    __builtin_amdgcn_wave_barrier();
#pragma unroll
                    for (int kt = 0; kt < 4; ++kt) {
#pragma unroll
                        for (int q = 0; q < 4; ++q) {
                            f32x4 v;
                            v[0] = x3[0][4 * half + kt][4 * q + 0];
                            v[1] = x3[0][4 * half + kt][4 * q + 1];
                            v[2] = x3[0][4 * half + kt][4 * q + 2];
                            v[3] = x3[0][4 * half + kt][4 * q + 3];
                            *reinterpret_cast<f32x4*>(s_x + (lane & 31) * HEAD_SCR_XLD + 32 * kt + 8 * q + 4 * h) = v;
                        }
                    }
                    __builtin_amdgcn_wave_barrier();
                    if (half == 1) HSCR_COUNT(4, (cnt + 63) / 64);
                    scr_recompute<HEAD_SCR_SW, 128 / HEAD_SCR_SW, HEAD_SCR_DEPTH, false>(
                        w.w4row + 128 * half, 256, s_list, cnt, s_x, HEAD_SCR_XLD, s_stage, lane,
                        [&](uint32_t idx, bool live) { return half == 0 ? 0.0f : s_part[live ? idx : 0u]; },
                        [&](float a, int c, uint32_t idx, bool live) {
                            if (half == 0) {
                                if (live) s_part[idx] = a;
                            } else {
                                int bits = __float_as_int(a + s_b4[c]);
                                bits = bits > 0 ? bits : 0;
                                if (live && bits > 0) atomicMax(&s_run[c], bits);
                            }
                        });
                    HSTAMP(4 + half);
                }
                HSTAMP_ADD(9, 1u);
            }
        }
        const bool more = ncur < n_live;
        const bool leave = !more || (int64_t)e[0] != b;
        if (leave) flush(b);
        HSTAMP(6);
        if (!more) break;
        if (leave) enter((int64_t)e[0]);
        HSTAMP(6);
        cur = ncur;
        run_end = nend;
#pragma unroll
        for (int k = 0; k < KS; ++k) in[0][k] = in_n[0][k];
    }
#ifdef DAL3_STAMP
    if (lane == 0 && blockIdx.x < 1024) {
#pragma unroll
        for (int k = 0; k < 10; ++k) g_head_stamps[blockIdx.x * 16 + k] = st_acc[k];
    }
#endif
}

hipError_t launch_point_head_screen(int head_kind, const PointHeadW& w, BCN x, int c_in, float* feat, uint32_t* ctl,
                                    const u32x4* list, int64_t max_tiles, int64_t slots, hipStream_t s) {
    if (!w.w4row || !w.w4h || !w.scr_pq || !w.scr_flag) return hipErrorInvalidValue;
    const dim3 grid((unsigned)(max_tiles < slots ? max_tiles : slots)), block(64);
    switch (head_kind) {
        case 1:
            hipLaunchKernelGGL((point_head_screen_kernel<2, 128, 128, 256>), grid, block, 0, s, w, x, c_in, feat, ctl, list);
            break;
        case 2:
            hipLaunchKernelGGL((point_head_screen_kernel<2, 64, 128, 256>), grid, block, 0, s, w, x, c_in, feat, ctl, list);
            break;
        default:
            return hipErrorInvalidValue;
    }
    return hipGetLastError();
}
```

### 3dal_pytorch_amd/csrc/dal3_kernels.h

```cpp
#pragma once
#include <hip/hip_runtime.h>
#include <stddef.h>
#include <stdint.h>

#include "../../include/dal3.h"
#include "dal3_device.h"
#include "dal3_fold.h"

#ifndef DAL3_ENC_T
#define DAL3_ENC_T 2
#endif
#ifndef DAL3_DEC_T
#define DAL3_DEC_T 1
#endif
#ifndef DAL3_HEAD_T
#define DAL3_HEAD_T 1
#endif

#ifndef DAL3_ENC_SCREEN
#define DAL3_ENC_SCREEN 1
#endif

#ifndef DAL3_WG_WAVES
#define DAL3_WG_WAVES 4
// ... 33 lines not shown
    const int32_t* scr_flag;
    const float* dw2c;
    const float* dw3c;
    const float* dw4c;
    const int32_t* dec_flag;
    const float* dw1c;
    const f32x4* w1h;
    const float* prn_pq;
    const uint32_t* dec_ident;
    const int32_t* prn_flag;
};
#ifndef DAL3_DEC_MIN_DEAD
#define DAL3_DEC_MIN_DEAD 64
#endif
#ifndef DAL3_DEC_PLAN_ROUND
#define DAL3_DEC_PLAN_ROUND 2
#endif
#define DEC_PLAN_LD 640
#define DEC_NULL_K 512
struct DecPlan {
    const uint32_t* k;
    const float* gbc;
    const int32_t* nch;
};
enum {
    ENC_W2 = 0, ENC_W3 = 16, ENC_W4 = 32, ENC_W5 = 64, ENC_FRAGS = 64 + 512,
    DEC_W2 = 0, DEC_MIX = 16, DEC_MIX_FRAGS = 8 + 16 * 40, DEC_W3 = 16 + 648, DEC_W4 = 16 + 648 + 128,
    DEC_FRAGS = 16 + 648 + 128 + 64,
    LAT_W1A = 0, LAT_W2 = 128, LAT_FRAGS = 128 + 512
};

struct PackGroups {
    int blocks = 0;
    int64_t a0 = 0, a1 = 0, stride = 0, last = -1;
};

struct FcW {
    const float* w[3];
    const float* b[3];
    int c_in[3], c_out[3], relu[3];
    int n;
};

struct PointHeadW {
    const float* w1;
    const float* b1;
    const float* b2;
    const float* b3;
    const float* b4;
    const f32x4* stream;
    FcW fc;
    const float* w4row;
    const f32x4* w4h;
    const float* scr_pq;
    const int32_t* scr_flag;
};

#define LP_ENC_SEG 32
#define LP_ENC_SEGS 9
#define LP_DEC_SEG 40
#define LP_DEC_SEGS 12
#define LP_HEAD_SEG 32
#ifndef DAL3_LP_ENC_T
#define DAL3_LP_ENC_T 4
#endif
#ifndef DAL3_LP_DEC_T
#define DAL3_LP_DEC_T 2
#endif
#ifndef DAL3_LP_HEAD_T
#define DAL3_LP_HEAD_T 2
#endif
struct InsSegLpW {
    const float* w1;
    const float* b1;
    const float* bias_enc;
    const float* bias_dec;
    const float* dw1g;
    const float* db1;
    const uint16_t* enc_stream;
    const uint16_t* dec_stream;
};
struct PointHeadLpW {
    const float* w1;
    const float* b1;
    const float* bias;
    const uint16_t* stream;
    FcW fc;
};
#ifndef DAL3_X3_HEAD_T
#define DAL3_X3_HEAD_T 2
#endif
#ifndef DAL3_X3_ENC_T
#define DAL3_X3_ENC_T 2
#endif
#ifndef DAL3_X3_DEC_T
#define DAL3_X3_DEC_T 2
#endif
typedef PointHeadLpW PointHeadX3W;
struct InsSegX3W {
    const float* w1;
    const float* b1;
    const float* bias_enc;
    const float* bias_dec;
    const float* dw1g;
    const float* db1;
    const uint16_t* enc_stream;
    const uint16_t* dec_stream;
};
hipError_t launch_ins_seg_encode_x3(const InsSegX3W& w, BCN pts, int c_in, int B, int N, float* g, hipStream_t s);
hipError_t launch_ins_seg_decode_x3(const InsSegX3W& w, BCN pts, int c_in, int B, int N, const float* gbias, float* logits,
                                    uint8_t* mask, hipStream_t s);
int point_head_x3_segments(int head_kind);
hipError_t launch_point_head_x3(int head_kind, const PointHeadX3W& w, BCN x, int c_in, int B, int M, float* feat,
                                const int32_t* distinct, hipStream_t s);
hipError_t launch_pack_weight_x3(const dal3_layer& L, int kt_major, int col_off, int n_cols, int mt_n, int kt_n, uint16_t* out,
                                 hipStream_t s, PackGroups G = PackGroups{});
hipError_t launch_ins_seg_encode_lp(int dtype, const InsSegLpW& w, BCN pts, int c_in, int B, int N, float* g, hipStream_t s);
hipError_t launch_ins_seg_decode_lp(int dtype, const InsSegLpW& w, BCN pts, int c_in, int B, int N, const float* gbias,
                                    float* logits, uint8_t* mask, hipStream_t s);
hipError_t launch_point_head_lp(int dtype, int head_kind, const PointHeadLpW& w, BCN x, int c_in, int B, int M,
                                float* feat, const int32_t* distinct, hipStream_t s);
hipError_t launch_pack_weight_lp(const dal3_layer& L, int dtype, int kt_major, int col_off, int n_cols, int mt_n, int kt_n,
                                 uint16_t* out, hipStream_t s, PackGroups G = PackGroups{});

void point_head_dims(int head_kind, int* c_in, int* ks, int c[4], int* n_fc, int fc_in[3], int fc_out[3]);

hipError_t launch_ins_seg_encode(const InsSegW& w, BCN pts, int c_in, int B, int N, float* g, hipStream_t s, uint32_t* prune = nullptr);
hipError_t launch_ins_seg_encode_screen(const InsSegW& w, BCN pts, int c_in, int B, int N, float* g, hipStream_t s, uint32_t* prune);
bool dec_plan_route(int flags, int B, int N);
int enc_route(int flags, int B, int N);
bool enc_resident_route(int flags, int B, int N);
hipError_t launch_pack_dec_prune(const dal3_layer& L, float* dw1c, float* pq, uint32_t* ident, int32_t* flag, hipStream_t s);
hipError_t launch_dec_plan(const InsSegW& w, const float* gb, const uint32_t* prune, int B, uint32_t* plan_k, float* plan_gbc,
                           int32_t* plan_nch, hipStream_t s);
hipError_t launch_pack_screen_bound(const dal3_layer& L, float* pq, int32_t* flag, hipStream_t s);
hipError_t launch_pack_dec_chain(const dal3_layer& L, const float* bias, float* wcopy, int32_t* flag, hipStream_t s);
hipError_t launch_ins_seg_decode(const InsSegW& w, BCN pts, int c_in, int B, int N, const float* gbias,
                                 float* logits, uint8_t* mask, hipStream_t s, DecPlan plan = DecPlan{nullptr, nullptr, nullptr});
size_t point_head_worklist_bytes(int B, int M);
hipError_t launch_point_head(int head_kind, const PointHeadW& w, BCN x, int c_in, int B, int M, float* feat,
                             const int32_t* distinct, hipStream_t s, void* worklist = nullptr, size_t worklist_bytes = 0);
#ifndef DAL3_HEAD_SCR_STRIDE
#define DAL3_HEAD_SCR_STRIDE 4
#endif
#ifndef DAL3_HEAD_SCREEN
#define DAL3_HEAD_SCREEN 1
#endif
#ifndef DAL3_HEAD_SCR_MIN_TILES
#define DAL3_HEAD_SCR_MIN_TILES 8192
#endif
static_assert(DAL3_HEAD_SCR_STRIDE >= 2, "stride 1 leaves no tile to screen");
hipError_t launch_point_head_screen(int head_kind, const PointHeadW& w, BCN x, int c_in, float* feat, uint32_t* ctl,
                                    const u32x4* list, int64_t max_tiles, int64_t slots, hipStream_t s);
hipError_t launch_pack_head_screen(const dal3_layer& L, float* pq, int32_t* flag, hipStream_t s);
hipError_t launch_generic_layer(const f32x4* wf, const float* w1, const float* bias, int kt_n, int ks_n, int mt_n,
                                int relu, BCN x, int c_in, int B, int N, float* y, hipStream_t s);

hipError_t launch_fc(const float* W, const float* bias, const float* x, int64_t xs, float* y, int64_t ys, int B,
                     int c_in, int c_out, int relu, hipStream_t s);

enum { PACK_FRAG_MT_MAJOR = 0, PACK_FRAG_KT_MAJOR = 1, PACK_FIRST = 2, PACK_ROWMAJOR = 3 };
hipError_t launch_pack_weight(const dal3_layer& L, int mode, int col_off, int n_cols, int mt_n, int kt_n, float* out,
                              hipStream_t s, PackGroups G = PackGroups{});
hipError_t launch_pack_bias(const dal3_layer& L, float* out, hipStream_t s);

hipError_t launch_static_crop_prep(const double* points, const int64_t* offsets, const int32_t* choice, const double* pose,
                                   const double* box, int B, int N, uint64_t seed, int64_t item_offset, float* pts_out,
                                   float* init_box_out, hipStream_t s);
hipError_t launch_dynamic_item_prep(const double* points, const int64_t* frame_offsets, const double* boxes,
                                    const int64_t* track_first, const int32_t* item_track, const int32_t* item_frame,
                                    const int32_t* choice, const double* pose, int B, int n_per, int r, int s_,
                                    uint64_t seed, int64_t item_offset, float* pts_out, float* box_out,
                                    float* init_box_out, hipStream_t st);
hipError_t launch_static_crop_labels(const double* points, const int64_t* offsets, const int32_t* choice, const double* pose,
                                     int B, int N, uint64_t seed, int64_t item_offset, const double* gt_planes,
                                     uint8_t* mask_label, hipStream_t s);
hipError_t launch_dynamic_item_labels(const double* points, const int64_t* frame_offsets, const int64_t* track_first,
                                      const int32_t* item_track, const int32_t* item_frame, const int32_t* choice,
                                      const double* pose, int B, int n_per, int r, uint64_t seed, int64_t item_offset,
                                      const double* xform, const double* planes, const uint8_t* valid, uint8_t* mask_label,
                                      hipStream_t st);
size_t crop_workspace_bytes(int64_t K_total, int64_t max_points_per_frame);
hipError_t launch_crop_count(const float* points, const int64_t* point_offsets, const double* planes,
                             const float* spheres, const int64_t* box_offsets, int F, int64_t K_total, int64_t max_points_per_frame,
                             int64_t* counts, int32_t* cc, hipStream_t s);
hipError_t launch_crop_fill(const float* points, const int64_t* point_offsets, const double* planes,
                            const float* spheres, const int64_t* box_offsets, int F, int64_t K_total,
                            int64_t max_points_per_frame, const double* pose, const int64_t* counts,
                            const int64_t* box_start, const int32_t* cc, double* out_points, int32_t* out_index,
                            int64_t out_capacity, hipStream_t s);
hipError_t launch_crop_starts(const int64_t* counts, const int64_t* order, int64_t K, int64_t* box_start, int64_t* out_offsets,
                              int64_t out_capacity, hipStream_t s);
int64_t box_iou_pairwise_blocks(int64_t n, int64_t m);
int64_t box_iou_paired_blocks(int64_t n);
hipError_t launch_box_iou_pairwise(const void* a, int64_t n, const void* b, int64_t m, int boxes_f64, float* iou_bev,
                                   float* iou_3d, hipStream_t s);
hipError_t launch_box_iou_paired(const void* a, const void* b, int64_t n, int boxes_f64, float* iou_bev, float* iou_3d,
                                 hipStream_t s);
int64_t box_estimation_metrics_chunks(int64_t N);
hipError_t launch_box_estimation_metrics(const dal3_box_metric_args* a, hipStream_t s);
size_t track_workspace_bytes(int64_t S, int64_t K, int64_t capacity);
size_t track_match_workspace_bytes(int64_t K);
hipError_t launch_track(const dal3_track_args* a, hipStream_t s);
hipError_t launch_track_match(const dal3_track_match_args* a, hipStream_t s);
size_t group_workspace_bytes(int64_t E, int64_t T);
size_t motion_classify_workspace_bytes(int64_t T);
hipError_t launch_group_by_key(const dal3_group_args* a, hipStream_t s);
hipError_t launch_track_features(const dal3_track_feature_args* a, hipStream_t s);
hipError_t launch_gt_table(const dal3_gt_table_args* a, hipStream_t s);
hipError_t launch_motion_classify(const dal3_motion_classify_args* a, hipStream_t s);
size_t score_workspace_bytes(int64_t S);
hipError_t launch_score_tracks(const dal3_score_args* a, hipStream_t s);
hipError_t launch_best_gt_iou(const dal3_best_gt_args* a, hipStream_t s);
size_t nms_workspace_bytes(int64_t K, int boxes_f64);
hipError_t launch_nms(const dal3_nms_args* a, hipStream_t s);
size_t center_decode_workspace_bytes(int64_t B, int64_t H, int64_t W);
hipError_t launch_center_decode(const dal3_center_decode_args* a, hipStream_t s);
hipError_t launch_center_decode_flip4(const dal3_center_decode_flip4_args* a, hipStream_t s);
hipError_t launch_flip4_points(const float* points, int64_t N, int C, const int64_t* offsets, int64_t B, float* out,
                               int64_t* out_offsets, int64_t max_workgroups, hipStream_t s);
size_t voxelize_workspace_bytes(int64_t B, int64_t N);
hipError_t launch_voxelize(const dal3_voxelize_args* a, hipStream_t s);
hipError_t launch_pillar_pack(const dal3_layer* layers, int n_layers, double eps, float* out, hipStream_t s);
hipError_t launch_pillar_features(const dal3_pillar_feature_args* a, hipStream_t s);
hipError_t launch_pillar_scatter(const float* features, const int32_t* coordinates, int64_t P, const int64_t* n_pillars, int c_out,
                                 float* canvas, int64_t canvas_B, int64_t ny, int64_t nx, hipStream_t s);
hipError_t launch_voxel_mean(const float* voxels, const int32_t* num_points, int64_t P, const int64_t* n_pillars, int max_points,
                             int C, float* out, hipStream_t s);
size_t conv2d_pack_floats(int kind, int c_in, int c_out);
hipError_t launch_conv2d_pack(const FoldLayer& layer, int kind, float* out, hipStream_t s);
hipError_t launch_conv2d(const dal3_conv2d_args* a, hipStream_t s);
size_t sp_sort_workspace_bytes(int64_t capacity);
hipError_t launch_sp_sort(const dal3_sp_sort_args* a, hipStream_t s);
int sp_candidates(const int32_t* kernel, const int32_t* stride);
size_t sp_downsample_workspace_bytes(int64_t in_capacity, int candidates);
hipError_t launch_sp_downsample(const dal3_sp_downsample_args* a, hipStream_t s);
hipError_t launch_sp_table(const dal3_sp_table_args* a, hipStream_t s);
size_t sp_conv_pack_floats(int taps, int c_in, int c_out);
hipError_t launch_sp_conv_pack(const FoldLayer& layer, int taps, float* out, int32_t* status, hipStream_t s);
hipError_t launch_sp_conv(const dal3_sp_conv_args* a, hipStream_t s);
hipError_t launch_sp_table_transposed(const dal3_sp_table_transposed_args* a, hipStream_t s);
size_t sp_wgrad_workspace_bytes(int taps, int c_in, int c_out, int64_t out_capacity);
hipError_t launch_sp_wgrad(const dal3_sp_wgrad_args* a, hipStream_t s);
hipError_t launch_points_in_boxes(const void* points, int points_f64, int64_t P, int64_t stride, const double* planes,
                                  int K, int f32_math, uint8_t* inside, hipStream_t s);
hipError_t launch_writeback(const double* final_boxes, const int32_t* final_idx, const double* pose_best,
                            const double* pose_inv, const double* track_box, float* det, const int64_t* det_start,
                            const int32_t* det_count, const uint8_t* active, int P, int64_t n_det, int32_t* match,
                            int32_t* owner, hipStream_t s);
hipError_t launch_maxpool_n(const void* x, int dtype, int64_t rows, int64_t n, void* out, hipStream_t s);
hipError_t launch_segment_counts(const uint8_t* mask, int B, int N, int32_t* counts, hipStream_t s);
hipError_t launch_fill_words(void* p, size_t n_words, uint32_t value, hipStream_t s);
hipError_t launch_nonfinite_rows(BCN x, int B, int n_pts, int c_in, float* dst, int C, hipStream_t s,
                                 const int32_t* distinct = nullptr, void* worklist = nullptr, int seed_stride = 0);
hipError_t launch_compact_sample(const uint8_t* mask, BCN pts, int B, int N, int C, int M, int sampler,
                                 const int32_t* choice, uint64_t seed, int64_t item_offset, int32_t* counts,
                                 int32_t* pos, int32_t* obj_idx, float* obj_pts, hipStream_t s, const int64_t* step = nullptr);
struct DecodeArgs {
    float* box_pred;
    const float* center_add;
    int64_t ca_stride;
    int center_inplace;
    const float* boxes_center_add;
    int64_t bca_stride;
    const float* yaw_base;
    int64_t yaw_stride;
    float* heading_residuals;
    float* size_residuals;
    float* center;
    float* boxes7;
};
hipError_t launch_fc39_decode(const float* W, const float* bias, const float* x, int64_t xs, int B, int c_in,
                              const DecodeArgs& d, hipStream_t s);
hipError_t launch_decode_boxes(float* box_pred, int B, const float* center_add, int64_t center_add_stride,
                               int center_inplace, const float* boxes_center_add, int64_t boxes_center_add_stride,
                               const float* yaw_base, int64_t yaw_stride, float* heading_residuals,
                               float* size_residuals, float* center, float* boxes7, hipStream_t s);
hipError_t launch_recenter(const float* obj_pts, int B, int M, const float* init_box7, const float* box_one7,
                           const float* bbox_gt7, float* obj_pts_two, int64_t* hcl, float* hrl, hipStream_t s);

hipError_t launch_tr_linear(const float* a, int64_t M, int c_in, int64_t lda, const float* scale, const float* shift,
                            int relu_in, const float* W, int64_t ldw, int transpose_w, const float* bias, int64_t seg,
                            int c_out, float* z, int64_t ldz, int accumulate, float* ws, hipStream_t s, bool prepacked = false);
size_t tr_linear_workspace_bytes(int c_in, int c_out);
int tr_linear_pack_mtb(int64_t M, int c_in, int64_t seg, int c_out, int accumulate, int has_act);
hipError_t launch_tr_pack_many(const dal3_tr_pack_item* items, int n, hipStream_t s);
int tr_linear_x3_layout(int64_t M, int c_in, int64_t seg, int c_out, int accumulate, int has_act);
hipError_t launch_tr_linear_x3(const float* a, int64_t M, int c_in, int64_t lda, const float* scale, const float* shift, int relu_in,
                               const uint16_t* wpk, int layout, const float* bias, int64_t seg, int c_out, float* z, int64_t ldz,
                               hipStream_t s, const uint32_t* in_amax = nullptr);
size_t tr_colred_workspace_bytes(int64_t M, int C);
hipError_t launch_tr_act_colsum(const float* x, int64_t M, int C, int64_t ldx, const float* scale, const float* shift, int relu,
                                float* out, int64_t ldo, double* part, double* sums, hipStream_t s);
hipError_t launch_tr_colred(const float* z, int64_t M, int C, int64_t ldz, int mode, const float* da, int64_t ldda,
                            const float* dg, const int32_t* arg, int64_t seg, const float* scale, const float* shift,
                            const float* mu, const float* rstd, double* part, double* out, hipStream_t s);
hipError_t launch_tr_pool_coef(const float* dg, const float* g, const float* zarg, const float* mu, const float* rstd,
                               const float* gamma, int B, int C, int64_t M, double* coef, float* kd, hipStream_t s);
hipError_t launch_tr_pool_moments(const float* W, int64_t ldw, const float* b, const double* m1, const float* Sc, int64_t M, int C,
                                  int K, double* sums, hipStream_t s);
__attribute__((visibility("hidden"))) bool tr_pool_k_ok(int K);
__attribute__((visibility("hidden"))) bool tr_conv1_ok(int c_in, int c_out);
size_t tr_pool_gv_workspace_bytes(int K);
hipError_t launch_tr_pool_gv(const double* coef, const float* W, int64_t ldw, const float* b, int C, int K, float* G, float* v,
                             double* ws, hipStream_t s);
hipError_t launch_tr_pool_dw(const double* coef, const float* W, int64_t ldw, const float* b, const float* S, const double* m1,
// ... 146 lines not shown
```

### 3dal_pytorch_amd/csrc/dal3_pointmlp.hip

```cpp
#include <stdlib.h>

#include <type_traits>

#include "dal3_device.h"
#include "dal3_kernels.h"

#ifdef DAL3_STAMP
__device__ long long* g_stamps = nullptr;
extern "C" int dal3_debug_set_stamps(void* p) {
    return (int)hipMemcpyToSymbol(HIP_SYMBOL(g_stamps), &p, sizeof(p));
}
#define STAMP(k)                                                                                  \
    do {                                                                                          \
        __builtin_amdgcn_sched_barrier(0);                                                        \
        unsigned long long t_;                                                                    \
        asm volatile("s_memtime %0\n\ts_waitcnt lgkmcnt(0)" : "=s"(t_)::"memory");               \
        __builtin_amdgcn_sched_barrier(0);                                                        \
        if (lane == 0 && blockIdx.x < 2048) g_stamps[(blockIdx.x * DAL3_WG_WAVES + wave) * 16 + (k)] = t_; \
    } while (0)
#else
#define STAMP(k)
#endif

#ifndef DAL3_ENC_LDS_MAX
// ... 700 lines not shown
            mlp_layer_ring<C2 / 32, C3 / 32, T>(ring, w.b3, w.b2, bias, x2, x3, lane);
            load_points<KS, T>(x, (int64_t)e[0], (int)e[1] * 32, (int)e[2], c_in, in_n, lane);
        }
        conv_max_layer<C3 / 32, T>(ring, s_b4, x3, reinterpret_cast<float*>(s_run), 16, lane);
        const bool more = ncur < n_live;
        if (!more || (int64_t)e[0] != b) flush(b);
        if (!more) break;
        cur = ncur;
        run_end = nend;
#pragma unroll
        for (int k = 0; k < KS; ++k) in[0][k] = in_n[0][k];
    }
}

__global__ __launch_bounds__(256) void generic_layer_kernel(const f32x4* __restrict__ wf, const float* __restrict__ w1,
                                                            const float* __restrict__ bias, int kt_n, int ks_n, int mt_n,
                                                            int relu, BCN x, int c_in, int n_pts, int tiles_per_item,
                                                            float* __restrict__ y) {
    const int lane = threadIdx.x & 63;
    const int wave = threadIdx.x >> 6;
    const int h = lane >> 5;
    const int64_t b = blockIdx.x / tiles_per_item;
    const int n0 = ((blockIdx.x % tiles_per_item) * 4 + wave) * 32;
    if (n0 >= n_pts) return;
    int n = n0 + (lane & 31);
    const bool valid = n < n_pts;
    n = valid ? n : n_pts - 1;
    const float* p = x.data + b * x.sb + (int64_t)n * x.sn;
    const int c_out = 32 * mt_n;
    for (int mt = 0; mt < mt_n; ++mt) {
        f32x16 acc = tile_from_channels(bias + 32 * mt, h);
        if (ks_n > 0) {
            for (int s = 0; s < ks_n; ++s) {
                const int c = 2 * s + h;
                const float bv = c < c_in ? p[c * x.sc] : 0.0f;
                acc = mfma32(w1[(mt * ks_n + s) * 64 + lane], bv, acc);
            }
        } else {
            for (int kt = 0; kt < kt_n; ++kt) {
                for (int q = 0; q < 4; ++q) {
                    const f32x4 a = wf[((mt * kt_n + kt) * 4 + q) * 64 + lane];
#pragma unroll
                    for (int e = 0; e < 4; ++e) {
                        const int c = 32 * kt + 8 * q + 4 * h + e;
                        acc = mfma32(a[e], p[c * x.sc], acc);
                    }
                }
            }
        }
        if (relu) acc = relu16(acc);
        if (valid) {
#pragma unroll
            for (int q = 0; q < 4; ++q) {
                f32x4 o;
                o[0] = acc[4 * q + 0];
                o[1] = acc[4 * q + 1];
                o[2] = acc[4 * q + 2];
                o[3] = acc[4 * q + 3];
                *reinterpret_cast<f32x4*>(y + (b * n_pts + n) * c_out + 32 * mt + 8 * q + 4 * h) = o;
            }
        }
    }
}

static inline int tiles_per_item(int n_pts, int T) {
    return (n_pts + 32 * DAL3_WG_WAVES * T - 1) / (32 * DAL3_WG_WAVES * T);
}

#ifndef DAL3_LAT_MAX_TILES
#define DAL3_LAT_MAX_TILES 512
#endif
#ifndef DAL3_LAT_MAX_TILES_ENC
#define DAL3_LAT_MAX_TILES_ENC DAL3_LAT_MAX_TILES
#endif
#ifndef DAL3_LAT_MAX_TILES_DEC
#define DAL3_LAT_MAX_TILES_DEC DAL3_LAT_MAX_TILES
#endif
#ifndef DAL3_LAT_MAX_TILES_HEAD
#define DAL3_LAT_MAX_TILES_HEAD DAL3_LAT_MAX_TILES
#endif
bool lat_use(int64_t tiles, int flags, int64_t max_tiles) { return !(flags & DAL3_BCN_NO_SMALL_JOB_KERNELS) && tiles <= max_tiles; }

bool dec_plan_route(int flags, int B, int N) {
    const int64_t tiles = (int64_t)B * ((N + 31) / 32);
    if (flags & DAL3_BCN_NO_DEC_PLAN) return false;
    if (!DAL3_ENC_SCREEN || !DAL3_DEC_SPARSE || DAL3_DEC_T != 1) return false;
    if (lat_use(tiles, flags, DAL3_LAT_MAX_TILES_ENC) || lat_use(tiles, flags, DAL3_LAT_MAX_TILES_DEC)) return false;
    return !(DAL3_ENC_T > 1 && (int64_t)B * N <= 1024 * 64);
}

#ifndef DAL3_ENC_RES_MIN_PER_CU
#define DAL3_ENC_RES_MIN_PER_CU 3
#endif
static int enc_cu_count() {
    static int n = 0;
    if (n == 0) {
        int dev = 0, v = 0;
        if (hipGetDevice(&dev) != hipSuccess || hipDeviceGetAttribute(&v, hipDeviceAttributeMultiprocessorCount, dev) != hipSuccess || v <= 0)
            v = 256;
        n = v;
    }
    return n;
}
bool enc_resident_route(int flags, int B, int N) {
    (void)N;
    return !(flags & DAL3_BCN_NO_ENC_RESIDENT) && (int64_t)B >= (int64_t)DAL3_ENC_RES_MIN_PER_CU * enc_cu_count();
}
int enc_route(int flags, int B, int N) {
    if (lat_use((int64_t)B * ((N + 31) / 32), flags, DAL3_LAT_MAX_TILES_ENC)) return DAL3_ENC_ROUTE_LATENCY;
    if (DAL3_ENC_T > 1 && (int64_t)B * N <= 1024 * 64) return DAL3_ENC_ROUTE_DENSE;
    if (!DAL3_ENC_SCREEN) return DAL3_ENC_ROUTE_DENSE;
    return enc_resident_route(flags, B, N) ? DAL3_ENC_ROUTE_RESIDENT : DAL3_ENC_ROUTE_TWO_LAUNCH;
}

hipError_t launch_ins_seg_encode(const InsSegW& w, BCN pts, int c_in, int B, int N, float* g, hipStream_t s, uint32_t* prune) {
    if (lat_use((int64_t)B * ((N + 31) / 32), pts.flags, DAL3_LAT_MAX_TILES_ENC)) return launch_ins_seg_encode_lat(w, pts, c_in, B, N, g, s);
    constexpr int T = DAL3_ENC_T;
    if (T > 1 && (int64_t)B * N <= 1024 * 64) {
        const int tpi1 = tiles_per_item(N, 1);
        hipLaunchKernelGGL(ins_seg_encode_kernel<1>, dim3((unsigned)((int64_t)B * tpi1)), dim3(64 * DAL3_WG_WAVES), 0, s, w, pts, c_in, N, tpi1, g);
        return hipGetLastError();
    }
    if (DAL3_ENC_SCREEN) return launch_ins_seg_encode_screen(w, pts, c_in, B, N, g, s, prune);
    const int tpi = tiles_per_item(N, T);
    hipLaunchKernelGGL(ins_seg_encode_kernel<T>, dim3((unsigned)((int64_t)B * tpi)), dim3(64 * DAL3_WG_WAVES), 0, s, w, pts, c_in, N, tpi, g);
    return hipGetLastError();
}

hipError_t launch_ins_seg_decode(const InsSegW& w, BCN pts, int c_in, int B, int N, const float* gbias,
                                 float* logits, uint8_t* mask, hipStream_t s, DecPlan plan) {
    if (lat_use((int64_t)B * ((N + 31) / 32), pts.flags, DAL3_LAT_MAX_TILES_DEC)) return launch_ins_seg_decode_lat(w, pts, c_in, B, N, gbias, logits, mask, s);
    constexpr int T = DAL3_DEC_T;
    const int tpi = tiles_per_item(N, T);
    constexpr size_t lds = DAL3_DEC_SPARSE != 0 && T == 1 ? (size_t)DAL3_WG_WAVES * DEC_Q_FLOATS * sizeof(float) : 0;
    if (lds) {
        const hipError_t e = hipFuncSetAttribute(reinterpret_cast<const void*>(ins_seg_decode_kernel<T>),
                                                 hipFuncAttributeMaxDynamicSharedMemorySize, (int)lds);
        if (e != hipSuccess) return e;
    }
    hipLaunchKernelGGL(ins_seg_decode_kernel<T>, dim3((unsigned)((int64_t)B * tpi)), dim3(64 * DAL3_WG_WAVES), lds, s, w, pts, c_in, N, tpi,
                       gbias, logits, mask, plan);
    return hipGetLastError();
}

size_t point_head_worklist_bytes(int B, int M) { return 256 + (size_t)B * ((M + 31) / 32) * sizeof(u32x4); }

static int head_slots() {
    int dev = 0, v = 0;
    if (hipGetDevice(&dev) != hipSuccess || hipDeviceGetAttribute(&v, hipDeviceAttributeMultiprocessorCount, dev) != hipSuccess || v <= 0)
        v = 256;
    return 4 * v;
}

hipError_t launch_point_head(int head_kind, const PointHeadW& w, BCN x, int c_in, int B, int M, float* feat,
                             const int32_t* distinct, hipStream_t s, void* worklist, size_t worklist_bytes) {
    constexpr int T = DAL3_HEAD_T;
    const int tpi = (M + 32 * T - 1) / (32 * T);
    const bool lat = lat_use((int64_t)B * ((M + 31) / 32), x.flags, DAL3_LAT_MAX_TILES_HEAD);
    const bool pers = !lat && worklist && worklist_bytes >= point_head_worklist_bytes(B, M) && !(x.flags & DAL3_BCN_NO_WORKLIST) && T == 1;
    const bool screen = DAL3_HEAD_SCREEN && pers && (head_kind == 1 || head_kind == 2) && w.w4row &&
                        (int64_t)B * tpi >= DAL3_HEAD_SCR_MIN_TILES && tpi > 1;
    hipError_t e0 = launch_nonfinite_rows(x, B, M, c_in, feat, 512, s, distinct, pers ? worklist : nullptr,
                                          screen ? DAL3_HEAD_SCR_STRIDE : 0);
    if (e0 != hipSuccess) return e0;
    if (lat) return launch_point_head_lat(head_kind, w, x, c_in, B, M, feat, distinct, s);
    if (pers) {
        uint32_t* ctl = static_cast<uint32_t*>(worklist);
        u32x4* list = reinterpret_cast<u32x4*>(static_cast<char*>(worklist) + 256);
        const int64_t slots = head_slots();
        const int64_t seed_tpi = (tpi + DAL3_HEAD_SCR_STRIDE - 1) / DAL3_HEAD_SCR_STRIDE;
        const int64_t tiles = screen ? (int64_t)B * seed_tpi : (int64_t)B * tpi;
        const dim3 grid((unsigned)(tiles < slots ? tiles : slots)), block(64);
        switch (head_kind) {
            case 1:
                hipLaunchKernelGGL((point_head_pers_kernel<2, 128, 128, 256>), grid, block, 0, s, w, x, c_in, feat, ctl, list);
                break;
            case 2:
                hipLaunchKernelGGL((point_head_pers_kernel<2, 64, 128, 256>), grid, block, 0, s, w, x, c_in, feat, ctl, list);
                break;
            case 3:
                hipLaunchKernelGGL((point_head_pers_kernel<4, 64, 64, 128>), grid, block, 0, s, w, x, c_in, feat, ctl, list);
                break;
            default:
                return hipErrorInvalidValue;
        }
        hipError_t e1 = hipGetLastError();
        if (e1 != hipSuccess || !screen) return e1;
        return launch_point_head_screen(head_kind, w, x, c_in, feat, ctl + 2, list + (size_t)B * seed_tpi,
                                        (int64_t)B * (tpi - seed_tpi), slots, s);
    }
    const dim3 grid((unsigned)((int64_t)B * tpi)), block(64);
    switch (head_kind) {
        case 1:
            hipLaunchKernelGGL((point_head_kernel<2, 128, 128, 256, T>), grid, block, 0, s, w, x, c_in, M, tpi, feat, distinct);
            break;
        case 2:
            hipLaunchKernelGGL((point_head_kernel<2, 64, 128, 256, T>), grid, block, 0, s, w, x, c_in, M, tpi, feat, distinct);
            break;
        case 3:
            hipLaunchKernelGGL((point_head_kernel<4, 64, 64, 128, T>), grid, block, 0, s, w, x, c_in, M, tpi, feat, distinct);
            break;
        default:
            return hipErrorInvalidValue;
    }
    return hipGetLastError();
}

hipError_t launch_generic_layer(const f32x4* wf, const float* w1, const float* bias, int kt_n, int ks_n, int mt_n,
                                int relu, BCN x, int c_in, int B, int N, float* y, hipStream_t s) {
    const int tpi = (N + 127) / 128;
    hipLaunchKernelGGL(generic_layer_kernel, dim3((unsigned)((int64_t)B * tpi)), dim3(256), 0, s, wf, w1, bias, kt_n,
                       ks_n, mt_n, relu, x, c_in, N, tpi, y);
    return hipGetLastError();
}
```

### include/dal3.h

```cpp
#ifndef DAL3_H
#define DAL3_H

#include <stddef.h>
#include <stdint.h>

#ifdef __cplusplus
extern "C" {
#endif

typedef void* dal3_stream;

#define DAL3_VERSION 170

enum {
    DAL3_OK = 0,
    DAL3_EINVAL = -1,
    DAL3_EWORKSPACE = -2,
    DAL3_EHIP = -3
};

#define DAL3_MAX_ITEMS 16777216
#define DAL3_MAX_POINTS_PER_ITEM 16777216
#define DAL3_MAX_TILES 2147483647

enum { DAL3_F32 = 0, DAL3_BF16 = 1, DAL3_F16 = 2,
       DAL3_F16X3 = 3 };

enum {
    DAL3_HEAD_INS_SEG = 0,
    DAL3_HEAD_STATIC_BOX_EST = 1,
    DAL3_HEAD_POINT_EMB = 2,
    DAL3_HEAD_BOX_EMB = 3,
    DAL3_HEAD_DYNAMIC_BOX_EST = 4
};

enum {
    DAL3_SAMPLER_DEVICE = 0,
    DAL3_SAMPLER_CHOICE = 1
};

typedef struct {
    const float* weight;
    const float* bias;
    const float* bn_weight;
    const float* bn_bias;
    const float* bn_mean;
    const float* bn_var;
    int32_t c_in;
    int32_t c_out;
} dal3_layer;

int dal3_version(void);
const char* dal3_last_error(void);
const float* dal3_mean_size(void);

int dal3_pack_weights(int head_kind, const dal3_layer* layers, int n_layers, int dtype,
                      void* packed_dev, size_t* bytes_inout, dal3_stream stream);

typedef struct {
    const float* data;
    int64_t stride_b, stride_c, stride_n;
    int32_t dtype;
    int32_t flags;
} dal3_bcn;

enum { DAL3_BCN_NO_SMALL_JOB_KERNELS = 1, DAL3_BCN_NO_WORKLIST = 2, DAL3_BCN_NO_LDS_SAMPLER = 4, DAL3_BCN_NO_DEC_PLAN = 16,
       DAL3_BCN_NO_ENC_RESIDENT = 32 };

size_t dal3_ins_seg_workspace_bytes(int B);
int dal3_ins_seg_plan_layout(int B, size_t off[4], int* min_dead);
enum { DAL3_ENC_ROUTE_LATENCY = 0, DAL3_ENC_ROUTE_DENSE = 1, DAL3_ENC_ROUTE_TWO_LAUNCH = 2, DAL3_ENC_ROUTE_RESIDENT = 3 };
int dal3_ins_seg_encoder_route(int B, int N, int flags);
int dal3_ins_seg_forward(const void* packed, int dtype, int c_in, dal3_bcn pts, int B, int N,
                         float* logits, uint8_t* mask, float* global_feat_out,
                         void* workspace, size_t workspace_bytes, dal3_stream stream);

int dal3_ins_seg_encode(const void* packed, int dtype, int c_in, dal3_bcn pts, int B, int N, float* global_feat,
                        dal3_stream stream);
int dal3_ins_seg_global_bias(const void* packed, int dtype, const float* global_feat, int B, float* gbias,
                             dal3_stream stream);
int dal3_ins_seg_decode(const void* packed, int dtype, int c_in, dal3_bcn pts, int B, int N, const float* gbias,
                        float* logits, uint8_t* mask, dal3_stream stream);

size_t dal3_gather_workspace_bytes(int B, int N);
int dal3_segment_counts(const uint8_t* mask, int B, int N, int32_t* counts, dal3_stream stream);
int dal3_mask_compact_sample(const uint8_t* mask, dal3_bcn pts, int B, int N, int C, int M,
                             int sampler, const int32_t* choice, uint64_t seed, int64_t item_offset,
                             int32_t* counts, int32_t* obj_idx, float* obj_pts,
                             void* workspace, size_t workspace_bytes, dal3_stream stream);

int dal3_mask_compact_sample_step(const uint8_t* mask, dal3_bcn pts, int B, int N, int C, int M, uint64_t seed,
                                  const int64_t* step, int64_t item_offset, int32_t* counts, int32_t* obj_idx,
                                  float* obj_pts, void* workspace, size_t workspace_bytes, dal3_stream stream);

size_t dal3_point_head_workspace_bytes(int B);
int dal3_point_head_forward(int head_kind, const void* packed, int dtype, dal3_bcn x, int B, int M,
                            float* out, int64_t out_stride,
                            void* workspace, size_t workspace_bytes, dal3_stream stream);

size_t dal3_point_head_pool_workspace_bytes(int B, int M);
int dal3_point_head_pool(int head_kind, const void* packed, int dtype, dal3_bcn x, int B, int M,
                         const int32_t* n_distinct, float* feat, void* workspace, size_t workspace_bytes,
                         dal3_stream stream);
int dal3_point_head_screen_min_tiles(void);
int dal3_point_head_screen_stride(void);

int dal3_dynamic_box_est_forward(const void* packed, const float* embedding, int B, float* box_pred,
                                 void* workspace, size_t workspace_bytes, dal3_stream stream);

int dal3_decode_boxes(float* box_pred, int B,
                      const float* center_add, int64_t center_add_stride, int center_inplace,
                      const float* boxes_center_add, int64_t boxes_center_add_stride,
                      const float* yaw_base, int64_t yaw_stride,
                      float* heading_residuals, float* size_residuals, float* center, float* boxes7,
                      dal3_stream stream);

int dal3_recenter_rotz(const float* obj_pts, int B, int M, const float* init_box7,
                       const float* box_one7, const float* bbox_gt7, float* obj_pts_two,
                       int64_t* heading_class_label, float* heading_residual_label,
                       dal3_stream stream);

int dal3_maxpool_n(const float* x, int64_t rows, int64_t n, float* out, dal3_stream stream);
int dal3_maxpool_n_dtype(const void* x, int dtype, int64_t rows, int64_t n, void* out, dal3_stream stream);

int dal3_static_crop_prep(const double* points, const int64_t* offsets, const int32_t* choice,
                          const double* pose, const double* box, int B, int N, uint64_t seed,
                          int64_t item_offset, float* pts_out, float* init_box_out, dal3_stream stream);

int dal3_dynamic_item_prep(const double* points, const int64_t* frame_offsets, const double* boxes,
                           const int64_t* track_first, const int32_t* item_track, const int32_t* item_frame,
                           const int32_t* choice, const double* pose, int B, int n_per, int r, int s,
                           uint64_t seed, int64_t item_offset, float* pts_out, float* box_out,
                           float* init_box_out, dal3_stream stream);

int dal3_writeback_boxes(const double* final_boxes, const int32_t* final_idx, const double* pose_best,
                         const double* pose_inv, const double* track_box, float* det, const int64_t* det_start,
                         const int32_t* det_count, const uint8_t* active, int P, int64_t n_det, int32_t* match,
                         int32_t* owner, dal3_stream stream);

int dal3_static_crop_labels(const double* points, const int64_t* offsets, const int32_t* choice, const double* pose,
                            int B, int N, uint64_t seed, int64_t item_offset, const double* gt_planes,
                            uint8_t* mask_label, dal3_stream stream);
int dal3_dynamic_item_labels(const double* points, const int64_t* frame_offsets, const int64_t* track_first,
                             const int32_t* item_track, const int32_t* item_frame, const int32_t* choice,
                             const double* pose, int B, int n_per, int r, uint64_t seed, int64_t item_offset,
                             const double* xform, const double* planes, const uint8_t* valid, uint8_t* mask_label,
                             dal3_stream stream);

int dal3_points_in_boxes(const void* points, int points_f64, int64_t P, int64_t stride, const double* planes, int K,
                         int f32_math, uint8_t* inside, dal3_stream stream);

int dal3_box_iou_pairwise(const void* a, int64_t n, const void* b, int64_t m, int boxes_f64, float* iou_bev,
                          float* iou_3d, dal3_stream stream);
int dal3_box_iou_paired(const void* a, const void* b, int64_t n, int boxes_f64, float* iou_bev, float* iou_3d,
                        dal3_stream stream);

enum { DAL3_BM_CENTER = 1, DAL3_BM_HEADING_SCORES = 2, DAL3_BM_HEADING_RESIDUALS = 4, DAL3_BM_SIZE_SCORES = 8,
       DAL3_BM_SIZE_RESIDUALS = 16, DAL3_BM_CENTER_LABEL = 32, DAL3_BM_HEADING_RESIDUAL_LABEL = 64,
       DAL3_BM_SIZE_RESIDUAL_LABEL = 128 };
enum { DAL3_BM_HEADING_CLASS_LABEL = 1, DAL3_BM_SIZE_CLASS_LABEL = 2 };
enum { DAL3_MASK_U8 = 0, DAL3_MASK_F32 = 1 };

typedef struct dal3_box_metric_acc {
    double sum_iou_bev;
    double sum_iou_3d;
    double sum_loss;
    uint64_t n_iou_3d_pass;
    uint64_t n_seg_correct;
    uint64_t n_items;
} dal3_box_metric_acc;

typedef struct dal3_box_metric_args {
    int64_t B, N;
    const void* center;                  int64_t ld_center;
    const void* heading_scores;          int64_t ld_heading_scores;
    const void* heading_residuals;       int64_t ld_heading_residuals;
    const void* size_scores;             int64_t ld_size_scores;
    const void* size_residuals;          int64_t ld_size_residuals;
    const void* center_label;            int64_t ld_center_label;
    const void* heading_class_label;     int64_t ld_heading_class_label;
    const void* heading_residual_label;  int64_t ld_heading_residual_label;
    const void* size_class_label;        int64_t ld_size_class_label;
    const void* size_residual_label;     int64_t ld_size_residual_label;
    int32_t f64_fields;
    int32_t i32_fields;
    const float* logits;
    int64_t logits_stride_b, logits_stride_n, logits_stride_c;
    const void* mask_label;
    int64_t mask_stride_b, mask_stride_n;
    int32_t mask_dtype;
    float thr;
    const float* loss;
    float* iou_bev;
    float* iou_3d;
    dal3_box_metric_acc* acc;
} dal3_box_metric_args;

int dal3_box_estimation_metrics(const dal3_box_metric_args* args, dal3_stream stream);

#define DAL3_TRACK_MAX_CAPACITY 65536
enum { DAL3_TRACK_OVERFLOW = 1, DAL3_TRACK_BAD_LABEL = 2, DAL3_TRACK_BAD_ID = 4 };

typedef struct dal3_track_args {
    int64_t S, F, K;
    const int64_t* seq_offsets;
    const int64_t* frame_offsets;
    const double* ct;
    const double* tracking;
    const int32_t* label;
    const float* score;
    float max_dist[3];
    int32_t max_age;
    double score_thresh;
    int64_t capacity;
    int32_t max_workgroups;
    int32_t reserved;
    const int64_t* id_base;
    int32_t* box_ids;
    int64_t* tracking_ids;
    int32_t* out_count;
    int64_t* id_total;
    int32_t* status;
    void* workspace;
    size_t workspace_bytes;
} dal3_track_args;

typedef struct dal3_track_match_args {
    int64_t F, K;
    const int64_t* frame_offsets;
    const int32_t* out_count;
    const int32_t* box_ids;
    const int64_t* tracking_ids;
    const int64_t* id_base;
    const float* boxes;
    const int64_t* gt_offsets;
    const float* gt_boxes;
    float thr;
    int32_t reserved;
    int32_t* match_frame;
    int32_t* match_obj;
    int32_t* status;
    void* workspace;
    size_t workspace_bytes;
} dal3_track_match_args;

size_t dal3_track_workspace_bytes(int64_t S, int64_t K, int64_t capacity);
int dal3_track(const dal3_track_args* args, dal3_stream stream);
size_t dal3_track_match_workspace_bytes(int64_t K);
int dal3_track_match(const dal3_track_match_args* args, dal3_stream stream);

enum { DAL3_MOTION_BAD_KEY = 8 };

typedef struct dal3_group_args {
    int64_t E, T, F;
    const int64_t* keys;
    const int64_t* key_base;
    int64_t key_bias;
    const int64_t* frame_offsets;
// ... 884 lines not shown
```

Before: 267,600 object-crops/s.

## Add resident point-head kernel holding one item per workgroup with LDS max table

Adds a new route for the static and embedding point heads. One 4-wave workgroup keeps a whole crop resident, carries the per-item max table in LDS, and pulls the next item from an atomic cursor. The first tile runs a screening pass to seed the bound, which replaces the two-launch screen and worklist path and its global atomics. The route is taken by default when B is large relative to the CU count, at the cost of more LDS per workgroup and a separate pre-pass sweep.

Result: faster. 274,200 object-crops/s (median of 6 runs) (+2.5%).

```diff
diff --git a/3dal_pytorch_amd/_hip.py b/3dal_pytorch_amd/_hip.py
--- a/3dal_pytorch_amd/_hip.py
+++ b/3dal_pytorch_amd/_hip.py
@@ -376,6 +376,7 @@
     "dal3_point_head_forward": (_i, [_i, vp, _i, BCN, _i, _i, vp, _i64, vp, _sz, vp]),
     "dal3_point_head_pool_workspace_bytes": (_sz, [_i, _i]),
     "dal3_point_head_screen_min_tiles": (_i, []),
+    "dal3_point_head_route": (_i, [_i, _i, _i, _i]),
     "dal3_point_head_screen_stride": (_i, []),
     "dal3_point_head_pool": (_i, [_i, vp, _i, BCN, _i, _i, vp, vp, vp, _sz, vp]),
     "dal3_dynamic_box_est_forward": (_i, [vp, vp, _i, vp, vp, _sz, vp]),
@@ -596,7 +597,9 @@
 BCN_NO_SMALL_JOB_KERNELS, BCN_NO_WORKLIST, BCN_NO_LDS_SAMPLER = 1, 2, 4
 BCN_NO_DEC_PLAN = 16
 BCN_NO_ENC_RESIDENT = 32
+BCN_NO_HEAD_RESIDENT = 64
 ENC_ROUTE_LATENCY, ENC_ROUTE_DENSE, ENC_ROUTE_TWO_LAUNCH, ENC_ROUTE_RESIDENT = 0, 1, 2, 3
+HEAD_ROUTE_LATENCY, HEAD_ROUTE_PER_TILE, HEAD_ROUTE_PERSISTENT, HEAD_ROUTE_TWO_LAUNCH, HEAD_ROUTE_RESIDENT = 0, 1, 2, 3, 4
 DISPATCH_FLAGS = 0
 
 
diff --git a/3dal_pytorch_amd/csrc/dal3_api.hip b/3dal_pytorch_amd/csrc/dal3_api.hip
--- a/3dal_pytorch_amd/csrc/dal3_api.hip
+++ b/3dal_pytorch_amd/csrc/dal3_api.hip
@@ -391,7 +391,7 @@
     if (t.dtype != DAL3_F32 && t.dtype != DAL3_BF16 && t.dtype != DAL3_F16)
         return fail(DAL3_EINVAL, "%s: storage dtype %d is none of DAL3_F32 / DAL3_BF16 / DAL3_F16", what, t.dtype);
     if (t.dtype != DAL3_F32 && (reinterpret_cast<uintptr_t>(t.data) & 1)) return fail(DAL3_EINVAL, "%s: 16-bit data must be 2-byte aligned", what);
-    if (t.flags & ~(DAL3_BCN_NO_SMALL_JOB_KERNELS | DAL3_BCN_NO_WORKLIST | DAL3_BCN_NO_LDS_SAMPLER | DAL3_BCN_NO_DEC_PLAN | DAL3_BCN_NO_ENC_RESIDENT)) return fail(DAL3_EINVAL, "%s: unknown bits in flags (%d)", what, t.flags);
+    if (t.flags & ~(DAL3_BCN_NO_SMALL_JOB_KERNELS | DAL3_BCN_NO_WORKLIST | DAL3_BCN_NO_LDS_SAMPLER | DAL3_BCN_NO_DEC_PLAN | DAL3_BCN_NO_ENC_RESIDENT | DAL3_BCN_NO_HEAD_RESIDENT)) return fail(DAL3_EINVAL, "%s: unknown bits in flags (%d)", what, t.flags);
     return 0;
 }
 
@@ -436,7 +436,7 @@
 
 extern "C" int dal3_ins_seg_encoder_route(int B, int N, int flags) {
     TRY(check_extent(B, N, "ins_seg_encoder_route"));
-    if (flags & ~(DAL3_BCN_NO_SMALL_JOB_KERNELS | DAL3_BCN_NO_WORKLIST | DAL3_BCN_NO_LDS_SAMPLER | DAL3_BCN_NO_DEC_PLAN | DAL3_BCN_NO_ENC_RESIDENT))
+    if (flags & ~(DAL3_BCN_NO_SMALL_JOB_KERNELS | DAL3_BCN_NO_WORKLIST | DAL3_BCN_NO_LDS_SAMPLER | DAL3_BCN_NO_DEC_PLAN | DAL3_BCN_NO_ENC_RESIDENT | DAL3_BCN_NO_HEAD_RESIDENT))
         return fail(DAL3_EINVAL, "ins_seg_encoder_route: unknown bits in flags (%d)", flags);
     return enc_route(flags, B, N);
 }
@@ -701,6 +701,13 @@
 
 extern "C" int dal3_point_head_screen_min_tiles(void) { return DAL3_HEAD_SCREEN ? DAL3_HEAD_SCR_MIN_TILES : 0x7fffffff; }
 extern "C" int dal3_point_head_screen_stride(void) { return DAL3_HEAD_SCR_STRIDE; }
+extern "C" int dal3_point_head_route(int head_kind, int B, int M, int flags) {
+    TRY(check_extent(B, M, "point_head_route"));
+    if (head_kind < 1 || head_kind > 3) return fail(DAL3_EINVAL, "point_head_route: unknown head kind %d", head_kind);
+    if (flags & ~(DAL3_BCN_NO_SMALL_JOB_KERNELS | DAL3_BCN_NO_WORKLIST | DAL3_BCN_NO_LDS_SAMPLER | DAL3_BCN_NO_DEC_PLAN | DAL3_BCN_NO_ENC_RESIDENT | DAL3_BCN_NO_HEAD_RESIDENT))
+        return fail(DAL3_EINVAL, "point_head_route: unknown bits in flags (%d)", flags);
+    return head_route(flags, head_kind, B, M);
+}
 
 extern "C" int dal3_dynamic_box_est_forward(const void* packed, const float* embedding, int B, float* box_pred,
                                             void* workspace, size_t workspace_bytes, dal3_stream stream) {
diff --git a/3dal_pytorch_amd/csrc/dal3_head_screen.hip b/3dal_pytorch_amd/csrc/dal3_head_screen.hip
--- a/3dal_pytorch_amd/csrc/dal3_head_screen.hip
+++ b/3dal_pytorch_amd/csrc/dal3_head_screen.hip
@@ -1,3 +1,4 @@
+#include <cstddef>
 #include "dal3_device.h"
 #include "dal3_kernels.h"
 #include "dal3_lp.h"
@@ -8,6 +9,9 @@
 #endif
 #define HEAD_SCR_XLD 132
 #define HEAD_SCR_SW 16
+#ifndef HEAD_RES_SW
+#define HEAD_RES_SW 32
+#endif
 #ifndef HEAD_SCR_DEPTH
 #define HEAD_SCR_DEPTH 1
 #endif
@@ -17,11 +21,12 @@
 #endif
 
 #ifdef DAL3_SCREEN_COUNT
-__device__ unsigned long long g_head_scr_count[8];
+#define HEAD_SCR_COUNTS 72
+__device__ unsigned long long g_head_scr_count[HEAD_SCR_COUNTS];
 extern "C" int dal3_debug_head_screen_counts(unsigned long long* out, int reset) {
     hipError_t e = hipMemcpyFromSymbol(out, HIP_SYMBOL(g_head_scr_count), sizeof(g_head_scr_count));
     if (e == hipSuccess && reset) {
-        unsigned long long z[8] = {};
+        unsigned long long z[HEAD_SCR_COUNTS] = {};
         e = hipMemcpyToSymbol(HIP_SYMBOL(g_head_scr_count), z, sizeof(z));
     }
     return (int)e;
@@ -35,6 +40,10 @@
 #endif
 
 #ifdef DAL3_STAMP
+struct HeadStamps {
+    uint32_t acc[12];
+    unsigned long long prev;
+};
 __device__ unsigned long long* g_head_stamps = nullptr;
 extern "C" int dal3_debug_set_head_stamps(void* p) {
     return (int)hipMemcpyToSymbol(HIP_SYMBOL(g_head_stamps), &p, sizeof(p));
@@ -49,14 +58,226 @@
     do {                                         \
         unsigned long long t_;                   \
         HSTAMP_NOW(t_);                          \
-        st_acc[k] += (uint32_t)(t_ - st_prev);   \
-        st_prev = t_;                            \
+        st.acc[k] += (uint32_t)(t_ - st.prev);   \
+        st.prev = t_;                            \
     } while (0)
-#define HSTAMP_ADD(k, v) st_acc[k] += (v)
+#define HSTAMP_ADD(k, v) st.acc[k] += (v)
 #else
+struct HeadStamps {};
 #define HSTAMP(k)
 #define HSTAMP_ADD(k, v)
 #endif
+
+template <int WAVES, int SW_ = HEAD_SCR_SW>
+struct HeadScreenLds {
+    static constexpr int SW = SW_;
+    f32x2 pq[512];
+    float b4[512];
+    int tab[512];
+    uint32_t list[WAVES * HEAD_SCR_CAP];
+    float part[WAVES * HEAD_SCR_CAP];
+    float x[WAVES * 32 * HEAD_SCR_XLD];
+    uint32_t stage[WAVES * 64 * (SW_ + 4)];
+    int g[WAVES == 1 ? 512 : 4];
+};
+using HeadResLds = HeadScreenLds<DAL3_WG_WAVES, HEAD_RES_SW>;
+static_assert(offsetof(HeadScreenLds<1>, x) % 16 == 0 && offsetof(HeadScreenLds<1>, stage) % 16 == 0 &&
+                  offsetof(HeadResLds, x) % 16 == 0 && offsetof(HeadResLds, stage) % 16 == 0 &&
+                  (32 * HEAD_SCR_XLD * 4) % 16 == 0 && (64 * (HEAD_SCR_SW + 4) * 4) % 16 == 0 && (64 * (HEAD_RES_SW + 4) * 4) % 16 == 0,
+              "x and stage are read and written 16 bytes at a time (the struct itself is placed on 16 bytes)");
+static_assert(4 * sizeof(HeadScreenLds<1>) <= 160 * 1024 && sizeof(HeadResLds) <= 160 * 1024 && DAL3_WG_WAVES == 4,
+              "the screened head's LDS exceeds a CU's 160 KiB: lower HEAD_SCR_CAP, HEAD_SCR_XLD or HEAD_SCR_SW");
+static_assert(16 * 64 <= 64 * (HEAD_SCR_SW + 4) && 16 * 64 <= 64 * (HEAD_RES_SW + 4), "the stage holds the hit words of conv4's 16 blocks");
+
+template <int PASS, bool OWN_G, class Lds>
+__device__ __forceinline__ void head_conv4_sweep(WRing<8>& r16, const ActTile<FP16> (&xh)[8], float X, uint32_t vmask, Lds& L,
+                                                 uint32_t* stage, ScreenHits<1>& hits, int lane) {
+    constexpr int KT = 8;
+    auto block_const = [&](int mt) -> float {
+        const int c = 32 * mt + (lane & 31);
+        const f32x2 pq = L.pq[c];
+        float E = fmaf(X, pq[0], pq[1]);
+        E = fmaf(E, 0x1p-20f, E);
+        if (PASS == 0) return E;
+        int gb = L.tab[c];
+        if (OWN_G) {
+            const int gs = L.g[c];
+            gb = gs > gb ? gs : gb;
+        }
+        const float G = __int_as_float(gb), bb = L.b4[c];
+        if (bits_nonfinite(G)) return 3.0e38f;
+        return (G - bb) - fmaf(__builtin_fabsf(G) + __builtin_fabsf(bb), 0x1p-22f, E);
+    };
+    uint32_t hb = 0;
+    float m = 0.0f;
+    auto ep_slice = [&](const f32x16& acc, int i, float k) {
+        if (PASS == 0) {
+            m = i == 0 ? __builtin_fmaxf(acc[0], acc[1]) : __builtin_fmaxf(__builtin_fmaxf(m, acc[2 * i]), acc[2 * i + 1]);
+        } else {
+            hb = scr_push_hit(hb, acc[2 * i], k);
+            hb = scr_push_hit(hb, acc[2 * i + 1], k);
+        }
+    };
+    auto ep_finish = [&](int mt, float k) {
+        if (PASS == 0) {
+            const int c = 32 * mt + (lane & 31);
+            m = __builtin_fmaxf(m, __shfl_xor(m, 32));
+            const float y = m - fmaf(__builtin_fabsf(m), 0x1p-22f, k);
+            int bits = __float_as_int(y + L.b4[c]);
+            bits = bits > 0 ? bits : 0;
+            if (lane < 32 && bits > 0) atomicMax(&L.tab[c], bits);
+        } else {
+            hits.park_block(stage, mt, hb & vmask, lane);
+        }
+    };
+    auto mm = [&](f32x16& acc, int mt, auto side) {
+        acc = f32x16{};
+#pragma unroll
+        for (int i = 0; i < 2 * KT; ++i) {
+            const f16x8_t a = __builtin_bit_cast(f16x8_t, r16.slot[i & 7]);
+            r16.slot[i & 7] = r16.fetch_at(((16u * (uint32_t)mt + (uint32_t)i + 8u) & 255u) * 1024u);
+            acc = FP16::mfma(xh[i >> 1].k[i & 1], a, acc);
+            DAL3_SCHED_FENCE();
+            side(i);
+            DAL3_SCHED_FENCE();
+        }
+    };
+    f32x16 accA, accB;
+    float kA = block_const(0), kB;
+    mm(accA, 0, NoSide());
+    int mt = 1;
+    for (; mt + 1 < 16; mt += 2) {
+        kB = block_const(mt);
+        mm(accB, mt, [&](int i) { if (i < 8) ep_slice(accA, i, kA); });
+        ep_finish(mt - 1, kA);
+        kA = block_const(mt + 1);
+        mm(accA, mt + 1, [&](int i) { if (i < 8) ep_slice(accB, i, kB); });
+        ep_finish(mt, kB);
+    }
+    kB = block_const(mt);
+    mm(accB, mt, [&](int i) { if (i < 8) ep_slice(accA, i, kA); });
+    ep_finish(mt - 1, kA);
+#pragma unroll
+    for (int i = 0; i < 8; ++i) ep_slice(accB, i, kB);
+    ep_finish(mt, kB);
+}
+
+template <bool RES, class Lds>
+__device__ __forceinline__ void head_screen_tile(const PointHeadW& w, const f32x4* w4f32, WRing<8>& r16, const f32x16 (&x3)[1][8],
+                                                 int e_t, int e_n, bool blob_dense, bool active, bool first, int round, Lds& L,
+                                                 int wave, int lane, HeadStamps& st) {
+    constexpr int T = 1, KT = 8;
+    const int h = lane >> 5;
+    uint32_t* const s_list = L.list + wave * HEAD_SCR_CAP;
+    float* const s_part = L.part + wave * HEAD_SCR_CAP;
+    float* const s_x = L.x + wave * 32 * HEAD_SCR_XLD;
+    uint32_t* const s_stage = L.stage + wave * 64 * (Lds::SW + 4);
+    auto dense_tile = [&]() {
+        WRing<DAL3_PF> r32;
+        r32.init(w4f32, lane);
+        conv_max_layer<KT, T>(r32, L.b4, x3, reinterpret_cast<float*>(L.tab), 16, lane);
+    };
+    bool dense = false;
+    if (active) {
+        int xm = 0;
+#pragma unroll
+        for (int kt = 0; kt < KT; ++kt) {
+#pragma unroll
+            for (int r = 0; r < 16; ++r) {
+                const int v = __float_as_int(x3[0][kt][r]);
+                xm = v > xm ? v : xm;
+            }
+        }
+        dense = blob_dense || __builtin_amdgcn_ballot_w64(xm > HEAD_SCR_XMAX_BITS) != 0;
+    }
+    const bool screened = active && !dense;
+    float X = 0.0f;
+    ActTile<FP16> xh[KT];
+    uint32_t vmask = 0;
+    if (screened) {
+        float ss = 0.0f;
+#pragma unroll
+        for (int kt = 0; kt < KT; ++kt) {
+#pragma unroll
+            for (int r = 0; r < 16; ++r) ss = fmaf(x3[0][kt][r], x3[0][kt][r], ss);
+        }
+        ss += __shfl_xor(ss, 32);
+#pragma unroll
+        for (int d = 16; d >= 1; d >>= 1) ss = __builtin_fmaxf(ss, __shfl_xor(ss, d));
+        X = sqrtf(ss) * (1.0f + 0x1p-15f);
+#pragma unroll
+        for (int kt = 0; kt < KT; ++kt) xh[kt] = pack_relu<FP16>(x3[0][kt]);
+        const int left = e_n - e_t * 32;
+#pragma unroll
+        for (int r = 0; r < 16; ++r) vmask |= tile_chan(r, h) < left ? (1u << (15 - r)) : 0u;
+        HSTAMP(1);
+    }
+    ScreenHits<T> hits;
+    hits.init();
+    if (RES && first) {
+        if (screened) head_conv4_sweep<0, false>(r16, xh, X, vmask, L, s_stage, hits, lane);
+        HSTAMP(10);
+        __syncthreads();
+        HSTAMP(11);
+    }
+    if (active && dense) {
+        HSCR_COUNT(1, 1);
+        dense_tile();
+        HSTAMP(7);
+    }
+    if (screened) {
+        head_conv4_sweep<1, !RES>(r16, xh, X, vmask, L, s_stage, hits, lane);
+        HSTAMP(2);
+        uint32_t cnt1[T];
+        const bool overflow = scr_build_lists<T, 16, HEAD_SCR_CAP>(s_stage, s_list, hits, cnt1, lane);
+        const uint32_t cnt = cnt1[0];
+        HSCR_COUNT(3, cnt);
+        if (RES) {
+            HSCR_COUNT(8 + (round < 31 ? round : 31), cnt);
+            HSCR_COUNT(40 + (round < 31 ? round : 31), 1);
+        }
+        HSTAMP(3);
+
+        if (overflow) {
+            HSCR_COUNT(2, 1);
+            dense_tile();
+            HSTAMP(7);
+        } else {
+#pragma unroll
+            for (int half = 0; half < 2; ++half) {
+                __builtin_amdgcn_wave_barrier();
+#pragma unroll
+                for (int kt = 0; kt < 4; ++kt) {
+#pragma unroll
+                    for (int q = 0; q < 4; ++q) {
+                        f32x4 v;
+                        v[0] = x3[0][4 * half + kt][4 * q + 0];
+                        v[1] = x3[0][4 * half + kt][4 * q + 1];
+                        v[2] = x3[0][4 * half + kt][4 * q + 2];
+                        v[3] = x3[0][4 * half + kt][4 * q + 3];
+                        *reinterpret_cast<f32x4*>(s_x + (lane & 31) * HEAD_SCR_XLD + 32 * kt + 8 * q + 4 * h) = v;
+                    }
+                }
+                __builtin_amdgcn_wave_barrier();
+                if (half == 1) HSCR_COUNT(4, (cnt + 63) / 64);
+                scr_recompute<Lds::SW, 128 / Lds::SW, HEAD_SCR_DEPTH, false>(
+                    w.w4row + 128 * half, 256, s_list, cnt, s_x, HEAD_SCR_XLD, s_stage, lane,
+                    [&](uint32_t idx, bool live) { return half == 0 ? 0.0f : s_part[live ? idx : 0u]; },
+                    [&](float a, int c, uint32_t idx, bool live) {
+                        if (half == 0) {
+                            if (live) s_part[idx] = a;
+                        } else {
+                            int bits = __float_as_int(a + L.b4[c]);
+                            bits = bits > 0 ? bits : 0;
+                            if (live && bits > 0) atomicMax(&L.tab[c], bits);
+                        }
+                    });
+                HSTAMP(4 + half);
+            }
+            HSTAMP_ADD(9, 1u);
+        }
+    }
+}
 
 template <int KS, int C1, int C2, int C3>
 __global__ __launch_bounds__(64) void point_head_screen_kernel(PointHeadW w, BCN x, int c_in, float* __restrict__ feat,
@@ -66,21 +287,11 @@
     static_assert(C3 == 256, "the bound, the two halves of k and the fp16 fragments are laid out for conv4 256 -> 512");
     const int lane = threadIdx.x & 63;
     const int h = lane >> 5;
-    __shared__ float s_b4[512];
-    __shared__ int s_run[512];
-    __shared__ int s_g[512];
-    __shared__ f32x2 s_pq[512];
-    __shared__ uint32_t s_list[HEAD_SCR_CAP];
-    __shared__ float s_part[HEAD_SCR_CAP];
-    __shared__ __attribute__((aligned(16))) float s_x[32 * HEAD_SCR_XLD];
-    __shared__ __attribute__((aligned(16))) uint32_t s_stage[64 * (HEAD_SCR_SW + 4)];
-    static_assert(4 * (3 * 512 * 4 + 512 * 8 + HEAD_SCR_CAP * 8 + 32 * HEAD_SCR_XLD * 4 + 64 * (HEAD_SCR_SW + 4) * 4) <= 160 * 1024,
-                  "the screened head's LDS exceeds a quarter of a CU's 160 KiB: lower HEAD_SCR_CAP, HEAD_SCR_XLD or HEAD_SCR_SW");
-    static_assert(16 * 64 <= 64 * (HEAD_SCR_SW + 4), "the stage holds the hit words of conv4's 16 blocks");
+    __shared__ __attribute__((aligned(16))) HeadScreenLds<1> L;
     for (int i = threadIdx.x; i < 512; i += 64) {
-        s_b4[i] = w.b4[i];
-        s_run[i] = 0;
-        s_pq[i] = reinterpret_cast<const f32x2*>(w.scr_pq)[i];
+        L.b4[i] = w.b4[i];
+        L.tab[i] = 0;
+        L.pq[i] = reinterpret_cast<const f32x2*>(w.scr_pq)[i];
     }
     __syncthreads();
     const uint32_t n_live = ctl[0];
@@ -103,27 +314,22 @@
     auto enter = [&](int64_t b) {
         const int* gi = reinterpret_cast<const int*>(feat + b * 512);
 #pragma unroll
-        for (int c = lane; c < 512; c += 64) s_g[c] = __hip_atomic_load(gi + c, __ATOMIC_RELAXED, __HIP_MEMORY_SCOPE_AGENT);
+        for (int c = lane; c < 512; c += 64) L.g[c] = __hip_atomic_load(gi + c, __ATOMIC_RELAXED, __HIP_MEMORY_SCOPE_AGENT);
     };
     auto flush = [&](int64_t b) {
         int* gi = reinterpret_cast<int*>(feat + b * 512);
 #pragma unroll
         for (int c = lane; c < 512; c += 64) {
-            const int v = s_run[c];
+            const int v = L.tab[c];
             if (v > 0) atomicMax(gi + c, v);
-            s_run[c] = 0;
-        }
-    };
-    auto dense_tile = [&](const f32x16 (&x3)[T][KT]) {
-        WRing<DAL3_PF> r32;
-        r32.init(w.stream + FRAGS23 * 64, lane);
-        conv_max_layer<KT, T>(r32, s_b4, x3, reinterpret_cast<float*>(s_run), 16, lane);
+            L.tab[c] = 0;
+        }
     };
     enter((int64_t)e[0]);
+    HeadStamps st;
 #ifdef DAL3_STAMP
-    uint32_t st_acc[10] = {};
-    unsigned long long st_prev;
-    HSTAMP_NOW(st_prev);
+    st = HeadStamps{};
+    HSTAMP_NOW(st.prev);
 #endif
     for (;;) {
         const int64_t b = (int64_t)e[0];
@@ -158,139 +364,7 @@
         HSCR_COUNT(0, 1);
         HSTAMP(0);
         HSTAMP_ADD(8, 1u);
-
-        int xm = 0;
-#pragma unroll
-        for (int kt = 0; kt < KT; ++kt) {
-#pragma unroll
-            for (int r = 0; r < 16; ++r) {
-                const int v = __float_as_int(x3[0][kt][r]);
-                xm = v > xm ? v : xm;
-            }
-        }
-        if (blob_dense || __builtin_amdgcn_ballot_w64(xm > HEAD_SCR_XMAX_BITS) != 0) {
-            HSCR_COUNT(1, 1);
-            dense_tile(x3);
-            HSTAMP(7);
-        } else {
-            float ss = 0.0f;
-#pragma unroll
-            for (int kt = 0; kt < KT; ++kt) {
-#pragma unroll
-                for (int r = 0; r < 16; ++r) ss = fmaf(x3[0][kt][r], x3[0][kt][r], ss);
-            }
-            ss += __shfl_xor(ss, 32);
-#pragma unroll
-            for (int d = 16; d >= 1; d >>= 1) ss = __builtin_fmaxf(ss, __shfl_xor(ss, d));
-            const float X = sqrtf(ss) * (1.0f + 0x1p-15f);
-
-            ActTile<FP16> xh[KT];
-#pragma unroll
-            for (int kt = 0; kt < KT; ++kt) xh[kt] = pack_relu<FP16>(x3[0][kt]);
-
-            ScreenHits<T> hits;
-            hits.init();
-            uint32_t vmask = 0;
-            {
-                const int left = e_n - e_t * 32;
-#pragma unroll
-                for (int r = 0; r < 16; ++r) vmask |= tile_chan(r, h) < left ? (1u << (15 - r)) : 0u;
-            }
-            HSTAMP(1);
-            auto block_const = [&](int mt) -> float {
-                const int c = 32 * mt + (lane & 31);
-                const f32x2 pq = s_pq[c];
-                float E = fmaf(X, pq[0], pq[1]);
-                E = fmaf(E, 0x1p-20f, E);
-                const int gs = s_g[c], gr = s_run[c];
-                const float G = __int_as_float(gs > gr ? gs : gr), bb = s_b4[c];
-                if (bits_nonfinite(G)) return 3.0e38f;
-                return (G - bb) - fmaf(__builtin_fabsf(G) + __builtin_fabsf(bb), 0x1p-22f, E);
-            };
-            uint32_t hb = 0;
-            auto ep_slice = [&](const f32x16& acc, int i, float k) {
-                hb = scr_push_hit(hb, acc[2 * i], k);
-                hb = scr_push_hit(hb, acc[2 * i + 1], k);
-            };
-            auto ep_finish = [&](int mt) {
-                hits.park_block(s_stage, mt, hb & vmask, lane);
-            };
-            auto mm = [&](f32x16& acc, int mt, auto side) {
-                acc = f32x16{};
-#pragma unroll
-                for (int i = 0; i < 2 * KT; ++i) {
-                    const f16x8_t a = __builtin_bit_cast(f16x8_t, r16.slot[i & 7]);
-                    r16.slot[i & 7] = r16.fetch_at(((16u * (uint32_t)mt + (uint32_t)i + 8u) & 255u) * 1024u);
-                    acc = FP16::mfma(xh[i >> 1].k[i & 1], a, acc);
-                    DAL3_SCHED_FENCE();
-                    side(i);
-                    DAL3_SCHED_FENCE();
-                }
-            };
-            f32x16 accA, accB;
-            float kA = block_const(0), kB;
-            mm(accA, 0, NoSide());
-            int mt = 1;
-            for (; mt + 1 < 16; mt += 2) {
-                kB = block_const(mt);
-                mm(accB, mt, [&](int i) { if (i < 8) ep_slice(accA, i, kA); });
-                ep_finish(mt - 1);
-                kA = block_const(mt + 1);
-                mm(accA, mt + 1, [&](int i) { if (i < 8) ep_slice(accB, i, kB); });
-                ep_finish(mt);
-            }
-            kB = block_const(mt);
-            mm(accB, mt, [&](int i) { if (i < 8) ep_slice(accA, i, kA); });
-            ep_finish(mt - 1);
-#pragma unroll
-            for (int i = 0; i < 8; ++i) ep_slice(accB, i, kB);
-            ep_finish(mt);
-            HSTAMP(2);
-            uint32_t cnt1[T];
-            const bool overflow = scr_build_lists<T, 16, HEAD_SCR_CAP>(s_stage, s_list, hits, cnt1, lane);
-            const uint32_t cnt = cnt1[0];
-            HSCR_COUNT(3, cnt);
-            HSTAMP(3);
-
-            if (overflow) {
-                HSCR_COUNT(2, 1);
-                dense_tile(x3);
-                HSTAMP(7);
-            } else {
-#pragma unroll
-                for (int half = 0; half < 2; ++half) {
-                    __builtin_amdgcn_wave_barrier();
-#pragma unroll
-                    for (int kt = 0; kt < 4; ++kt) {
-#pragma unroll
-                        for (int q = 0; q < 4; ++q) {
-                            f32x4 v;
-                            v[0] = x3[0][4 * half + kt][4 * q + 0];
-                            v[1] = x3[0][4 * half + kt][4 * q + 1];
-                            v[2] = x3[0][4 * half + kt][4 * q + 2];
-                            v[3] = x3[0][4 * half + kt][4 * q + 3];
-                            *reinterpret_cast<f32x4*>(s_x + (lane & 31) * HEAD_SCR_XLD + 32 * kt + 8 * q + 4 * h) = v;
-                        }
-                    }
-                    __builtin_amdgcn_wave_barrier();
-                    if (half == 1) HSCR_COUNT(4, (cnt + 63) / 64);
-                    scr_recompute<HEAD_SCR_SW, 128 / HEAD_SCR_SW, HEAD_SCR_DEPTH, false>(
-                        w.w4row + 128 * half, 256, s_list, cnt, s_x, HEAD_SCR_XLD, s_stage, lane,
-                        [&](uint32_t idx, bool live) { return half == 0 ? 0.0f : s_part[live ? idx : 0u]; },
-                        [&](float a, int c, uint32_t idx, bool live) {
-                            if (half == 0) {
-                                if (live) s_part[idx] = a;
-                            } else {
-                                int bits = __float_as_int(a + s_b4[c]);
-                                bits = bits > 0 ? bits : 0;
-                                if (live && bits > 0) atomicMax(&s_run[c], bits);
-                            }
-                        });
-                    HSTAMP(4 + half);
-                }
-                HSTAMP_ADD(9, 1u);
-            }
-        }
+        head_screen_tile<false>(w, w.stream + FRAGS23 * 64, r16, x3, e_t, e_n, blob_dense, true, false, 0, L, 0, lane, st);
         const bool more = ncur < n_live;
         const bool leave = !more || (int64_t)e[0] != b;
         if (leave) flush(b);
@@ -306,9 +380,106 @@
 #ifdef DAL3_STAMP
     if (lane == 0 && blockIdx.x < 1024) {
 #pragma unroll
-        for (int k = 0; k < 10; ++k) g_head_stamps[blockIdx.x * 16 + k] = st_acc[k];
-    }
-#endif
+        for (int k = 0; k < 10; ++k) g_head_stamps[blockIdx.x * 16 + k] = st.acc[k];
+    }
+#endif
+}
+
+template <int KS, int C1, int C2, int C3>
+__global__ __launch_bounds__(64 * DAL3_WG_WAVES) void point_head_resident_kernel(PointHeadW w, BCN x, int c_in, int n_pts,
+                                                                                float* __restrict__ feat,
+                                                                                const int32_t* __restrict__ distinct, int B,
+                                                                                uint32_t* __restrict__ cursor) {
+    constexpr int T = 1;
+    constexpr int KT = C3 / 32;
+    static_assert(C3 == 256, "the bound, the two halves of k and the fp16 fragments are laid out for conv4 256 -> 512");
+    const int lane = threadIdx.x & 63;
+    const int wave = __builtin_amdgcn_readfirstlane((int)(threadIdx.x >> 6));
+    const int h = lane >> 5;
+    __shared__ __attribute__((aligned(16))) HeadResLds L;
+    __shared__ int s_item;
+    for (int i = threadIdx.x; i < 512; i += 64 * DAL3_WG_WAVES) {
+        L.b4[i] = w.b4[i];
+        L.pq[i] = reinterpret_cast<const f32x2*>(w.scr_pq)[i];
+    }
+    const bool blob_dense = *w.scr_flag != 0;
+    constexpr uint32_t FRAGS23 = ((C2 / 32) * (C1 / 32) + (C3 / 32) * (C2 / 32)) * 4u;
+    WRing<DAL3_PF, true> ring;
+    ring.init(w.stream, lane, FRAGS23 * 1024u);
+    WRing<8> r16;
+    r16.init(w.w4h, lane);
+    f32x16 bias = tile_from_channels(w.b2, h);
+    HeadStamps st;
+#ifdef DAL3_STAMP
+    st = HeadStamps{};
+    HSTAMP_NOW(st.prev);
+#endif
+    for (int64_t b = blockIdx.x;;) {
+        int* const gi = reinterpret_cast<int*>(feat + b * 512);
+        int i0 = threadIdx.x;
+        asm volatile("" : "+v"(i0));
+        for (int i = i0; i < 512; i += 64 * DAL3_WG_WAVES) L.tab[i] = gi[i];
+        __syncthreads();
+        int n_eff = n_pts;
+        if (distinct) {
+            const int d = distinct[b];
+            n_eff = d <= 0 ? 1 : (d < n_pts ? d : n_pts);
+        }
+        const int n_t = (n_eff + 31) >> 5, R = (n_t + DAL3_WG_WAVES - 1) / DAL3_WG_WAVES;
+        float in[T][KS];
+        load_points<KS, T>(x, b, R * wave * 32, n_eff, c_in, in, lane);
+        for (int r = 0; r < R; ++r) {
+            const int t = r + R * wave;
+            const bool active = t < n_t;
+            f32x16 x3[T][KT];
+            if (active) {
+                f32x16 x1[T][C1 / 32], x2[T][C2 / 32];
+                first_layer<KS, C1 / 32, T>(w.w1, w.b1, in, x1, lane);
+                mlp_layer_ring<C1 / 32, C2 / 32, T>(ring, w.b2, w.b3, bias, x1, x2, lane);
+                mlp_layer_ring<C2 / 32, C3 / 32, T>(ring, w.b3, w.b2, bias, x2, x3, lane);
+                load_points<KS, T>(x, b, (t + 1) * 32, n_eff, c_in, in, lane);
+                HSCR_COUNT(0, 1);
+                HSTAMP(0);
+                HSTAMP_ADD(8, 1u);
+            }
+            head_screen_tile<true>(w, w.stream + FRAGS23 * 64, r16, x3, t, n_eff, blob_dense, active, r == 0, r, L, wave, lane, st);
+        }
+        __syncthreads();
+        i0 = threadIdx.x;
+        asm volatile("" : "+v"(i0));
+        for (int c = i0; c < 512; c += 64 * DAL3_WG_WAVES) gi[c] = L.tab[c];
+        HSTAMP(6);
+        if (threadIdx.x == 0) s_item = (int)(atomicAdd(cursor, 1u) + gridDim.x);
+        __syncthreads();
+        b = __builtin_amdgcn_readfirstlane(s_item);
+        if (b >= B) break;
+    }
+#ifdef DAL3_STAMP
+    if (lane == 0 && blockIdx.x * DAL3_WG_WAVES + wave < 1024) {
+#pragma unroll
+        for (int k = 0; k < 12; ++k) g_head_stamps[(blockIdx.x * DAL3_WG_WAVES + wave) * 16 + k] = st.acc[k];
+    }
+#endif
+}
+
+hipError_t launch_point_head_resident(int head_kind, const PointHeadW& w, BCN x, int c_in, int B, int M, float* feat,
+                                      const int32_t* distinct, hipStream_t s, void* cursor, int cus) {
+    if (!w.w4row || !w.w4h || !w.scr_pq || !w.scr_flag || !cursor || B < 1 || cus < 1) return hipErrorInvalidValue;
+    const hipError_t e0 = hipMemsetAsync(cursor, 0, sizeof(uint32_t), s);
+    if (e0 != hipSuccess) return e0;
+    const dim3 grid((unsigned)(B < cus ? B : cus)), block(64 * DAL3_WG_WAVES);
+    uint32_t* const cur = static_cast<uint32_t*>(cursor);
+    switch (head_kind) {
+        case 1:
+            hipLaunchKernelGGL((point_head_resident_kernel<2, 128, 128, 256>), grid, block, 0, s, w, x, c_in, M, feat, distinct, B, cur);
+            break;
+        case 2:
+            hipLaunchKernelGGL((point_head_resident_kernel<2, 64, 128, 256>), grid, block, 0, s, w, x, c_in, M, feat, distinct, B, cur);
+            break;
+        default:
+            return hipErrorInvalidValue;
+    }
+    return hipGetLastError();
 }
 
 hipError_t launch_point_head_screen(int head_kind, const PointHeadW& w, BCN x, int c_in, float* feat, uint32_t* ctl,
diff --git a/3dal_pytorch_amd/csrc/dal3_kernels.h b/3dal_pytorch_amd/csrc/dal3_kernels.h
--- a/3dal_pytorch_amd/csrc/dal3_kernels.h
+++ b/3dal_pytorch_amd/csrc/dal3_kernels.h
@@ -209,6 +209,10 @@
 static_assert(DAL3_HEAD_SCR_STRIDE >= 2, "stride 1 leaves no tile to screen");
 hipError_t launch_point_head_screen(int head_kind, const PointHeadW& w, BCN x, int c_in, float* feat, uint32_t* ctl,
                                     const u32x4* list, int64_t max_tiles, int64_t slots, hipStream_t s);
+bool head_resident_route(int flags, int head_kind, int B, int M);
+int head_route(int flags, int head_kind, int B, int M);
+hipError_t launch_point_head_resident(int head_kind, const PointHeadW& w, BCN x, int c_in, int B, int M, float* feat,
+                                      const int32_t* distinct, hipStream_t s, void* cursor, int cus);
 hipError_t launch_pack_head_screen(const dal3_layer& L, float* pq, int32_t* flag, hipStream_t s);
 hipError_t launch_generic_layer(const f32x4* wf, const float* w1, const float* bias, int kt_n, int ks_n, int mt_n,
                                 int relu, BCN x, int c_in, int B, int N, float* y, hipStream_t s);
diff --git a/3dal_pytorch_amd/csrc/dal3_pointmlp.hip b/3dal_pytorch_amd/csrc/dal3_pointmlp.hip
--- a/3dal_pytorch_amd/csrc/dal3_pointmlp.hip
+++ b/3dal_pytorch_amd/csrc/dal3_pointmlp.hip
@@ -876,17 +876,41 @@
     return 4 * v;
 }
 
+#ifndef DAL3_HEAD_RES_MIN_PER_CU
+#define DAL3_HEAD_RES_MIN_PER_CU 3
+#endif
+#ifndef DAL3_HEAD_RES_MIN_PER_CU_EMB
+#define DAL3_HEAD_RES_MIN_PER_CU_EMB 4
+#endif
+bool head_resident_route(int flags, int head_kind, int B, int M) {
+    if (!DAL3_HEAD_SCREEN || DAL3_HEAD_T != 1 || (flags & (DAL3_BCN_NO_HEAD_RESIDENT | DAL3_BCN_NO_WORKLIST))) return false;
+    if ((head_kind != 1 && head_kind != 2) || (M + 31) / 32 <= 1) return false;
+    if (lat_use((int64_t)B * ((M + 31) / 32), flags, DAL3_LAT_MAX_TILES_HEAD)) return false;
+    return (int64_t)B >= (int64_t)(head_kind == 1 ? DAL3_HEAD_RES_MIN_PER_CU : DAL3_HEAD_RES_MIN_PER_CU_EMB) * (head_slots() / 4);
+}
+int head_route(int flags, int head_kind, int B, int M) {
+    const int64_t tiles = (int64_t)B * ((M + 31) / 32);
+    if (lat_use(tiles, flags, DAL3_LAT_MAX_TILES_HEAD)) return DAL3_HEAD_ROUTE_LATENCY;
+    if ((flags & DAL3_BCN_NO_WORKLIST) || DAL3_HEAD_T != 1) return DAL3_HEAD_ROUTE_PER_TILE;
+    if (head_resident_route(flags, head_kind, B, M)) return DAL3_HEAD_ROUTE_RESIDENT;
+    if (DAL3_HEAD_SCREEN && (head_kind == 1 || head_kind == 2) && tiles >= DAL3_HEAD_SCR_MIN_TILES && (M + 31) / 32 > 1)
+        return DAL3_HEAD_ROUTE_TWO_LAUNCH;
+    return DAL3_HEAD_ROUTE_PERSISTENT;
+}
+
 hipError_t launch_point_head(int head_kind, const PointHeadW& w, BCN x, int c_in, int B, int M, float* feat,
                              const int32_t* distinct, hipStream_t s, void* worklist, size_t worklist_bytes) {
     constexpr int T = DAL3_HEAD_T;
     const int tpi = (M + 32 * T - 1) / (32 * T);
     const bool lat = lat_use((int64_t)B * ((M + 31) / 32), x.flags, DAL3_LAT_MAX_TILES_HEAD);
     const bool pers = !lat && worklist && worklist_bytes >= point_head_worklist_bytes(B, M) && !(x.flags & DAL3_BCN_NO_WORKLIST) && T == 1;
-    const bool screen = DAL3_HEAD_SCREEN && pers && (head_kind == 1 || head_kind == 2) && w.w4row &&
+    const bool resident = pers && w.w4row && head_resident_route(x.flags, head_kind, B, M);
+    const bool screen = DAL3_HEAD_SCREEN && pers && !resident && (head_kind == 1 || head_kind == 2) && w.w4row &&
                         (int64_t)B * tpi >= DAL3_HEAD_SCR_MIN_TILES && tpi > 1;
-    hipError_t e0 = launch_nonfinite_rows(x, B, M, c_in, feat, 512, s, distinct, pers ? worklist : nullptr,
+    hipError_t e0 = launch_nonfinite_rows(x, B, M, c_in, feat, 512, s, distinct, pers && !resident ? worklist : nullptr,
                                           screen ? DAL3_HEAD_SCR_STRIDE : 0);
     if (e0 != hipSuccess) return e0;
+    if (resident) return launch_point_head_resident(head_kind, w, x, c_in, B, M, feat, distinct, s, worklist, head_slots() / 4);
     if (lat) return launch_point_head_lat(head_kind, w, x, c_in, B, M, feat, distinct, s);
     if (pers) {
         uint32_t* ctl = static_cast<uint32_t*>(worklist);
diff --git a/include/dal3.h b/include/dal3.h
--- a/include/dal3.h
+++ b/include/dal3.h
@@ -65,7 +65,7 @@
 } dal3_bcn;
 
 enum { DAL3_BCN_NO_SMALL_JOB_KERNELS = 1, DAL3_BCN_NO_WORKLIST = 2, DAL3_BCN_NO_LDS_SAMPLER = 4, DAL3_BCN_NO_DEC_PLAN = 16,
-       DAL3_BCN_NO_ENC_RESIDENT = 32 };
+       DAL3_BCN_NO_ENC_RESIDENT = 32, DAL3_BCN_NO_HEAD_RESIDENT = 64 };
 
 size_t dal3_ins_seg_workspace_bytes(int B);
 int dal3_ins_seg_plan_layout(int B, size_t off[4], int* min_dead);
@@ -104,6 +104,9 @@
                          dal3_stream stream);
 int dal3_point_head_screen_min_tiles(void);
 int dal3_point_head_screen_stride(void);
+enum { DAL3_HEAD_ROUTE_LATENCY = 0, DAL3_HEAD_ROUTE_PER_TILE = 1, DAL3_HEAD_ROUTE_PERSISTENT = 2, DAL3_HEAD_ROUTE_TWO_LAUNCH = 3,
+       DAL3_HEAD_ROUTE_RESIDENT = 4 };
+int dal3_point_head_route(int head_kind, int B, int M, int flags);
 
 int dal3_dynamic_box_est_forward(const void* packed, const float* embedding, int B, float* box_pred,
                                  void* workspace, size_t workspace_bytes, dal3_stream stream);
```
